# PickNikRobotics/pick_ik

Measured on AMD Instinct MI355X. Metric: converged IK solves/sec (7-DOF Panda, batched random targets), higher is better.
Workload: dtype f64; 1 GPU; panda 7-DOF memetic IK (BASELINE configs[1]): population 128, elites 4, batch 4096 random reachable targets per GPU per step, seed = ready pose, max_generations 100, gd_max_iters 25; robot=panda, dof=7, tip_frames=1, batch_per_gpu=4096, batches_per_call=64, calls=21, streams=4, problems_in_flight_per_gpu=1048576, parallelism=shard1, arithmetic=exact

## Files before the change

include/pick_ik_amd.h:

```cpp
#ifndef PICK_IK_AMD_H
#define PICK_IK_AMD_H

#include <stdint.h>

#ifdef __cplusplus
extern "C" {
#endif

#define PIKAMD_MAX_DOF 16

#define PIKAMD_SUCCESS 1
#define PIKAMD_APPROXIMATE 2
#define PIKAMD_NO_IK_SOLUTION (-31)

#define PIKAMD_EINVAL (-1)
#define PIKAMD_ENODEVICE (-2)
#define PIKAMD_EHIP (-3)
#define PIKAMD_EUNSUPPORTED (-4)

#define PIKAMD_JOINT_REVOLUTE 0
#define PIKAMD_JOINT_PRISMATIC 1
#define PIKAMD_JOINT_PLANAR_X 2
#define PIKAMD_JOINT_PLANAR_Y 3
#define PIKAMD_JOINT_PLANAR_THETA 4
#define PIKAMD_JOINT_FLOATING_TX 5
#define PIKAMD_JOINT_FLOATING_TY 6
#define PIKAMD_JOINT_FLOATING_TZ 7
#define PIKAMD_JOINT_FLOATING_RX 8
#define PIKAMD_JOINT_FLOATING_RY 9
#define PIKAMD_JOINT_FLOATING_RZ 10
#define PIKAMD_JOINT_FLOATING_RW 11

typedef struct pikamd_chain {
    int32_t dof;
    const double* origin_xyz_rpy;
    const double* axis;
    const int32_t* joint_type;
    const double* tip_xyz_rpy;
    const double* qmin;
    const double* qmax;
    const double* vmax;
    const uint8_t* bounded;
} pikamd_chain;

#define PIKAMD_MAX_TIPS 8
typedef struct pikamd_tip {
    int32_t n_joints;
    const int32_t* variable;
    const double* origin_xyz_rpy;
    const double* axis;
    const int32_t* joint_type;
    const double* tip_xyz_rpy;
} pikamd_tip;
typedef struct pikamd_multi_chain {
    int32_t dof;
    int32_t n_tips;
    const pikamd_tip* tips;
    const double* qmin;
    const double* qmax;
    const double* vmax;
    const uint8_t* bounded;
} pikamd_multi_chain;

typedef struct pikamd_params {
    int32_t mode;
    double gd_step_size;
    int32_t gd_max_iters;
    double gd_min_cost_delta;
    double position_threshold;
    double orientation_threshold;
    double cost_threshold;
    double position_scale;
    double rotation_scale;
    double center_joints_weight;
    double avoid_joint_limits_weight;
    double minimal_displacement_weight;
    int32_t stop_optimization_on_valid_solution;
    int32_t memetic_num_threads;
    int32_t memetic_stop_on_first_solution;
    int32_t memetic_population_size;
    int32_t memetic_elite_size;
    double memetic_wipeout_fitness_tol;
    int32_t memetic_max_generations;
    int32_t memetic_gd_max_iters;
    int32_t return_approximate_solution;
} pikamd_params;

typedef struct pikamd_stats {
    int64_t cost_evals;
    int32_t generations;
    int32_t wipeouts;
    int32_t pool_erasures;
    int32_t reserved;
} pikamd_stats;

typedef struct pikamd_solver pikamd_solver;

void pikamd_default_params(pikamd_params* p);

int32_t pikamd_create(const pikamd_chain* chain, int32_t device_ordinal, pikamd_solver** out);
int32_t pikamd_create_multi(const pikamd_multi_chain* chain, int32_t device_ordinal,
                            pikamd_solver** out);
int32_t pikamd_n_tips(const pikamd_solver* s);

#define PIKAMD_MAX_MIMIC 4
typedef struct pikamd_mimic_joint {
    int32_t tip;
    int32_t after_variable;
    int32_t master_variable;
    int32_t joint_type;
    double origin_xyz_rpy[6];
    double axis[3];
    double multiplier, offset;
} pikamd_mimic_joint;
int32_t pikamd_set_mimic_joints(pikamd_solver* s, int32_t n, const pikamd_mimic_joint* joints);
void pikamd_destroy(pikamd_solver* s);
int32_t pikamd_variables(const pikamd_solver* s, double* out);

int32_t pikamd_fk_batch(pikamd_solver* s, int64_t n, const double* q, double* pos_quat);

int32_t pikamd_cost_batch(pikamd_solver* s, const pikamd_params* p, int64_t n,
                          const double* goal_pos_quat, const double* seed, const double* q,
                          double* cost, int32_t* is_solution);

int32_t pikamd_gd_step_batch(pikamd_solver* s, const pikamd_params* p, int64_t n,
                             const double* goal_pos_quat, const double* seed, double* local,
                             double* best, double* local_cost, double* best_cost,
                             double* gradient, int32_t* improved);

int32_t pikamd_solve_batch(pikamd_solver* s, const pikamd_params* p, int64_t B,
                           const double* goal_pos_quat, const double* seed, uint64_t rng_seed,
                           int64_t problem_offset, double* solution, int32_t* status,
                           double* final_cost, pikamd_stats* stats);

#define PIKAMD_MAX_SLOTS 128
int32_t pikamd_solve_batch_device(pikamd_solver* s, const pikamd_params* p, int64_t B,
                                  const double* d_goal_pos_quat, const double* d_seed,
                                  uint64_t rng_seed, int64_t problem_offset, double* d_solution,
                                  int32_t* d_status, double* d_final_cost, pikamd_stats* d_stats,
                                  void* stream, int32_t slot);
int32_t pikamd_fk_batch_device(pikamd_solver* s, int64_t n, const double* d_q, double* d_pos_quat,
                               void* stream);
int32_t pikamd_reserve(pikamd_solver* s, const pikamd_params* p, int64_t B, int32_t slot,
                       void* stream);

#define PIKAMD_MAX_BATCHES 64
typedef struct pikamd_batch {
    int64_t B;
    const double* goal_pos_quat;
    const double* seed;
    const double* initial_guess;
    int64_t problem_offset;
    double* solution;
    int32_t* status;
    double* final_cost;
    pikamd_stats* stats;
    uint32_t* completed;
} pikamd_batch;

int32_t pikamd_solve_batches_device(pikamd_solver* s, const pikamd_params* p, int32_t n_batches,
                                    const pikamd_batch* batches, uint64_t rng_seed, void* stream,
                                    int32_t slot);

#define PIKAMD_MAX_HOST_JOBS 16
int32_t pikamd_solve_batches_async(pikamd_solver* s, const pikamd_params* p, int32_t n_batches,
                                   const pikamd_batch* batches, uint64_t rng_seed, int32_t job);
int32_t pikamd_wait(pikamd_solver* s, int32_t job);
int32_t pikamd_solve_batches(pikamd_solver* s, const pikamd_params* p, int32_t n_batches,
                             const pikamd_batch* batches, uint64_t rng_seed);

void pikamd_shard_bounds(int64_t total, int32_t rank, int32_t world, int64_t* lo, int64_t* hi);
int32_t pikamd_solve_batch_sharded(pikamd_solver* const* solvers, int32_t n_devices, const pikamd_params* p,
                                   int64_t B, const double* goal_pos_quat, const double* seed,
                                   const double* initial_guess , uint64_t rng_seed,
                                   int64_t problem_offset, double* solution, int32_t* status,
                                   double* final_cost , pikamd_stats* stats );

#define PIKAMD_MAX_NAME 64
typedef struct pikamd_urdf_model {
    int32_t dof, n_tips;
    char variable_names[PIKAMD_MAX_DOF][PIKAMD_MAX_NAME];
    double qmin[PIKAMD_MAX_DOF], qmax[PIKAMD_MAX_DOF], vmax[PIKAMD_MAX_DOF];
    uint8_t bounded[PIKAMD_MAX_DOF];
    struct {
        int32_t n_joints;
        int32_t variable[PIKAMD_MAX_DOF];
        double origin_xyz_rpy[PIKAMD_MAX_DOF][6];
        double axis[PIKAMD_MAX_DOF][3];
        int32_t joint_type[PIKAMD_MAX_DOF];
        double tip_xyz_rpy[6];
    } tips[PIKAMD_MAX_TIPS];
    int32_t n_mimic;
    pikamd_mimic_joint mimic[PIKAMD_MAX_TIPS * PIKAMD_MAX_MIMIC];
} pikamd_urdf_model;
int32_t pikamd_urdf_extract(const char* urdf_xml, const char* base_link, const char* const* tip_links,
                            int32_t n_tips, pikamd_urdf_model* out);
int32_t pikamd_create_from_urdf(const char* urdf_xml, const char* base_link, const char* const* tip_links,
                                int32_t n_tips, int32_t device_ordinal, pikamd_solver** out);

typedef double (*pikamd_cost_fn)(const double* q, int32_t dof, int32_t pose_index, void* user);
int32_t pikamd_solve_batch_host(pikamd_solver* s, const pikamd_params* p, int64_t B, const double* goal_pos_quat,
                                const double* seed, const double* initial_guess, uint64_t rng_seed,
                                int64_t problem_offset, pikamd_cost_fn cost_fn, void* user, double* solution,
                                int32_t* status, double* final_cost, pikamd_stats* stats);

int32_t pikamd_set_option(pikamd_solver* s, const char* name, const char* value);

int32_t pikamd_self_test(pikamd_solver* s, const pikamd_params* p, int32_t n, uint32_t* disabled_mask);
int32_t pikamd_self_test_cost(const pikamd_solver* s, int32_t* runs, double* total_ms);

const char* pikamd_last_error(void);
const char* pikamd_version(void);
const char* pikamd_kernel_name(const pikamd_solver* s, const pikamd_params* p);

#define PIKAMD_NOT_ATTEMPTED 0
#define PIKAMD_PATH_JUMP (-1001)
int32_t pikamd_solve_paths(pikamd_solver* s, const pikamd_params* p, int64_t P, int32_t W,
                           const double* goal_pos_quat, const double* start, const double* max_joint_step,
                           double* solution, int32_t* status, double* final_cost, pikamd_stats* stats,
                           int32_t* reached);
int32_t pikamd_solve_paths_device(pikamd_solver* s, const pikamd_params* p, int64_t P, int32_t W,
                                  const double* d_goal_pos_quat, const double* d_start,
                                  const double* d_max_joint_step, double* d_solution, int32_t* d_status,
                                  double* d_final_cost, pikamd_stats* d_stats, int32_t* d_reached,
                                  void* stream, int32_t slot);
const char* pikamd_path_kernel_name(const pikamd_solver* s, const pikamd_params* p, int64_t P);

#define PIKAMD_MAX_ATTEMPTS 64
int32_t pikamd_search_batch(pikamd_solver* s, const pikamd_params* p, int64_t B, const double* goal_pos_quat,
                            const double* seed, const double* initial_guess, uint64_t rng_seed,
                            int64_t problem_offset, int32_t max_attempts, double* solution, int32_t* status,
                            double* final_cost, pikamd_stats* stats, int32_t* attempts, double* all_solution,
                            int32_t* all_status);
int32_t pikamd_search_batch_device(pikamd_solver* s, const pikamd_params* p, int64_t B,
                                   const double* d_goal_pos_quat, const double* d_seed,
                                   const double* d_initial_guess, uint64_t rng_seed, int64_t problem_offset,
                                   int32_t max_attempts, double* d_solution, int32_t* d_status,
                                   double* d_final_cost, pikamd_stats* d_stats, int32_t* d_attempts,
                                   double* d_all_solution, int32_t* d_all_status, void* stream, int32_t slot);
const char* pikamd_search_kernel_name(const pikamd_solver* s, const pikamd_params* p, int64_t B,
                                      int32_t max_attempts, int32_t* attempts_in_flight);

#ifdef __cplusplus
}
#endif
#endif
```

pick_ik_amd/build.py:

```python
from __future__ import annotations

import concurrent.futures as cf
import hashlib
import os
import re
import shutil
import subprocess

_HERE = os.path.dirname(os.path.abspath(__file__))
CSRC = os.path.join(_HERE, "csrc")
LIB = os.path.join(_HERE, "libpick_ik_amd.so")
LIB_STRICT = os.path.join(_HERE, "libpick_ik_amd_strict.so")
HEADERS = ["pik_kernels.hpp", "pik_math.hpp", "pik_host.hpp", "pik_solver.hpp", "pik_launch.hpp", "pik_exact.hpp",
           "pik_host_solve.hpp", "pik_path.hpp", "pik_path_ops.hpp", "pik_search.hpp", "pik_search_ops.hpp"]
HEADER = os.path.join(os.path.dirname(_HERE), "include", "pick_ik_amd.h")
DOFS = tuple(range(1, 17))
BUILD_DIR = os.path.join(_HERE, "_build")


def hipcc() -> str:
    for cand in (shutil.which("hipcc"), "/opt/rocm/bin/hipcc"):
        if cand and os.path.exists(cand):
            return cand
    raise RuntimeError("hipcc not found")


COMMON_FLAGS = ["-DPIK_COMMON=1"]
COMMON_GOALS_FLAGS = ["-DPIK_COMMON=1", "-DPIK_NO_GOALS=0"]


def _flavor_flags(strict: bool):
    flags = ["-DPIK_STRICT=1", "-ffp-contract=off"] if strict else ["-ffp-contract=on"]
    return flags + os.environ.get("PIK_EXTRA_HIPCC_FLAGS", "").split()


def _objects(strict: bool):
    d = os.path.join(BUILD_DIR, "strict" if strict else "fast")
    only = os.environ.get("PIK_ONLY_D")
    keep = {int(x) for x in only.split(",")} if only else set(DOFS)
    objs = [(os.path.join(d, "pik_amd.o"), "pik_amd.hip", [])]
    objs.append((os.path.join(d, "pik_host_solve.o"), "pik_host_solve.hip",
                 ["--cuda-host-only"] + ([] if strict else EXACT_FLAGS)))
    for n in DOFS:
        extra = [f"-DPIK_INST_D={n}"] + ([] if n in keep else ["-DPIK_INST_STUB=1"])
        objs.append((os.path.join(d, f"pik_inst_d{n}.o"), "pik_inst.hip", extra))
    return objs


def _is_strict_obj(o) -> bool:
    return os.sep + "strict" + os.sep in o[0]


EXACT_FLAGS = ["-DPIK_STRICT=1", "-DPIK_EXACT_FMA=1", "-ffp-contract=off"]


def _exact_objects():
    d = os.path.join(BUILD_DIR, "exact")
    only = os.environ.get("PIK_ONLY_D")
    keep = {int(x) for x in only.split(",")} if only else set(DOFS)
    return [(os.path.join(d, f"pik_inst_d{n}.o"), "pik_inst.hip",
             [f"-DPIK_INST_D={n}"] + (EXACT_FLAGS if n in keep else ["-DPIK_INST_STUB=1"] + EXACT_FLAGS)) for n in DOFS]


def _is_exact_obj(o) -> bool:
    return os.sep + "exact" + os.sep in o[0]


def _path_objects(flavour: str):
    d = os.path.join(BUILD_DIR, flavour)
    fl = EXACT_FLAGS if flavour == "exact" else []
    only = os.environ.get("PIK_ONLY_D")
    keep = {int(x) for x in only.split(",")} if only else set(DOFS)
    return [(os.path.join(d, f"pik_path_inst_d{n}.o"), "pik_path_inst.hip",
             [f"-DPIK_INST_D={n}"] + (fl if n in keep else ["-DPIK_INST_STUB=1"] + fl)) for n in DOFS]


def _search_objects(flavour: str):
    d = os.path.join(BUILD_DIR, flavour)
    fl = EXACT_FLAGS if flavour == "exact" else []
    only = os.environ.get("PIK_ONLY_D")
    keep = {int(x) for x in only.split(",")} if only else set(DOFS)
    return [(os.path.join(d, f"pik_search_inst_d{n}.o"), "pik_search_inst.hip",
             [f"-DPIK_INST_D={n}"] + (fl if n in keep else ["-DPIK_INST_STUB=1"] + fl)) for n in DOFS]


def _common_objects(goals: bool = False):
    d = os.path.join(BUILD_DIR, "common_goals" if goals else "common")
    fl = COMMON_GOALS_FLAGS if goals else COMMON_FLAGS
    only = os.environ.get("PIK_ONLY_D")
    keep = {int(x) for x in only.split(",")} if only else set(DOFS)
    return [(os.path.join(d, f"pik_inst_d{n}.o"), "pik_inst.hip",
             [f"-DPIK_INST_D={n}"] + (fl if n in keep else ["-DPIK_INST_STUB=1"] + fl)) for n in DOFS]


def _cmd(obj, src, extra, strict):
    bare = "-DPIK_EXACT_FMA=1" in extra
    flavour = os.environ.get("PIK_EXTRA_HIPCC_FLAGS", "").split() if bare else _flavor_flags(strict)
    return [hipcc(), "--offload-arch=gfx950", "--offload-compress", "-O2", "-std=c++17", "-fPIC", "-c", *flavour,
            "-Rpass-analysis=kernel-resource-usage", *extra, "-o", obj, os.path.join(CSRC, src)]


def _stamp(cmd):
    return hashlib.sha1(" ".join(cmd).encode()).hexdigest()


def _obj_stale(obj, src, extra, strict) -> bool:
    if not os.path.exists(obj) or not os.path.exists(obj + ".cmd"):
        return True
    if open(obj + ".cmd").read() != _stamp(_cmd(obj, src, extra, strict)):
        return True
    deps = _deps(src, "-DPIK_STRICT=1" in _cmd(obj, src, extra, strict))
    if os.path.exists(obj + ".deps"):
        return open(obj + ".deps").read() != _code_hash(deps)
    t = os.path.getmtime(obj)
    if any(os.path.getmtime(d) > t for d in deps):
        return True
    with open(obj + ".deps", "w") as f:
        f.write(_code_hash(deps))
    return False


def _strip_comments(text: str) -> str:
    out, i, n = [], 0, len(text)
    while i < n:
        c = text[i]
        if c == '"' or c == "'":
            j = i + 1
            while j < n and text[j] != c:
                j += 2 if text[j] == "\\" else 1
            out.append(text[i:j + 1])
            i = j + 1
        elif text.startswith("//", i):
            j = text.find("\n", i)
            i = n if j < 0 else j
        elif text.startswith("/*", i):
            j = text.find("*/", i + 2)
            i = n if j < 0 else j + 2
            out.append(" ")
        else:
            out.append(c)
            i += 1
    return " ".join("".join(out).split())


_code_hash_cache = {}


def _code_hash(files) -> str:
    h = hashlib.sha1()
    for f in files:
        key = (f, os.path.getmtime(f))
        if key not in _code_hash_cache:
            _code_hash_cache[key] = hashlib.sha1(_strip_comments(open(f).read()).encode()).hexdigest()
        h.update(_code_hash_cache[key].encode())
    return h.hexdigest()


_INCLUDE = re.compile(r'^\s*#\s*include\s+"([^"]+)"', re.M)


def _deps(src, strict_flags: bool):
    seen, todo = [], [os.path.join(CSRC, src)]
    while todo:
        f = os.path.realpath(todo.pop())
        if f in seen or not os.path.exists(f):
            continue
        seen.append(f)
        for inc in _INCLUDE.findall(open(f).read()):
            if os.path.basename(inc) == "pik_exact.hpp" and not strict_flags:
                continue
            todo.append(os.path.join(os.path.dirname(f), inc))
    return seen


def _sources():
    return ([os.path.join(CSRC, f) for f in ("pik_amd.hip", "pik_inst.hip", "pik_path_inst.hip", "pik_search_inst.hip", "pik_urdf.hpp",
                                             *HEADERS)] +
            [HEADER, os.path.abspath(__file__)])


def _lib_stamp(strict: bool) -> str:
    flags = _flavor_flags(strict) + ([] if strict else ["+exact:"] + EXACT_FLAGS + ["+common:"] + COMMON_FLAGS + ["+common_goals:"] + COMMON_GOALS_FLAGS)
    return _stamp(flags + ["+paths", "+search", "only=" + os.environ.get("PIK_ONLY_D", "all")])


def is_stale(lib: str = LIB) -> bool:
    if not os.path.exists(lib) or not os.path.exists(lib + ".stamp"):
        return True
    if open(lib + ".stamp").read() != _lib_stamp(lib == LIB_STRICT):
        return True
    t = os.path.getmtime(lib)
    return any(os.path.getmtime(d) > t for d in _sources())


def _compile(obj, src, extra, strict, verbose):
    os.makedirs(os.path.dirname(obj), exist_ok=True)
    cmd = _cmd(obj, src, extra, strict)
    if verbose:
        print(" ".join(cmd), flush=True)
    r = subprocess.run(cmd, cwd=CSRC, stderr=subprocess.PIPE, text=True)
    if r.returncode != 0:
        raise RuntimeError(f"{' '.join(cmd)}\n{r.stderr[-4000:]}")
    with open(obj + ".res", "w") as f:
        f.write(r.stderr)
    with open(obj + ".cmd", "w") as f:
        f.write(_stamp(cmd))
    with open(obj + ".deps", "w") as f:
        f.write(_code_hash(_deps(src, "-DPIK_STRICT=1" in cmd)))


def _link(lib, objs, verbose):
    cmd = [hipcc(), "--offload-arch=gfx950", "-shared", "-fPIC", "-o", lib + ".tmp", *objs]
    if verbose:
        print(" ".join(cmd), flush=True)
    subprocess.run(cmd, check=True)
    os.replace(lib + ".tmp", lib)


FLAVOUR_FLAGS = {
    "pik": ["-ffp-contract=on"],
    "pik_common": ["-ffp-contract=on"] + COMMON_FLAGS,
    "pik_common_goals": ["-ffp-contract=on"] + COMMON_GOALS_FLAGS,
    "pik_exact": EXACT_FLAGS,
    "pik_strict": ["-DPIK_STRICT=1", "-ffp-contract=off"],
}
_flavour_sha_cache = {}


def _host_api_lines():
    out, inside = set(), False
    for n, line in enumerate(open(HEADER).read().splitlines(), 1):
        if "[host-api-begin]" in line:
            inside = True
        if inside:
            out.add(n)
        if "[host-api-end]" in line:
            inside = False
    return out


def flavour_sha(namespace: str, dof: int = 7) -> str:
    key = (namespace, dof)
    if key in _flavour_sha_cache:
        return _flavour_sha_cache[key]
    flags = FLAVOUR_FLAGS[namespace]
    cmd = [hipcc(), "--offload-arch=gfx950", "-std=c++17", "--cuda-device-only", "-E", *flags, f"-DPIK_INST_D={dof}",
           os.path.join(CSRC, "pik_inst.hip"), "-o", "-"]
    r = subprocess.run(cmd, cwd=CSRC, stdout=subprocess.PIPE, stderr=subprocess.PIPE, text=True)
    if r.returncode != 0:
        raise RuntimeError(f"{' '.join(cmd)}\n{r.stderr[-2000:]}")
    own = (os.path.realpath(CSRC) + os.sep, os.path.realpath(HEADER))
    host_api = _host_api_lines()
    h = hashlib.sha256(" ".join(flags).encode())
    keep, in_header, lineno = False, False, 0
    for line in r.stdout.splitlines():
        if line.startswith("# ") and '"' in line:
            f = line.split('"')[1]
            rp = os.path.realpath(f if os.path.isabs(f) else os.path.join(CSRC, f))
            keep = rp.startswith(own[0]) or rp == own[1]
            in_header = rp == own[1]
            lineno = int(line.split()[1])
            continue
        if keep and line.strip() and not (in_header and lineno in host_api):
            h.update(line.strip().encode())
            h.update(b"\n")
        lineno += 1
    _flavour_sha_cache[key] = h.hexdigest()[:16]
    return _flavour_sha_cache[key]


LEDGER = os.path.join(BUILD_DIR, "kernel_resources.csv")


def ledger_rows():
    from . import kernel_resources as KR
    rows = []
    for o in (_objects(False) + _exact_objects() + _common_objects() + _common_objects(True) + _objects(True) +
              _path_objects("fast") + _path_objects("exact") + _path_objects("strict") +
              _search_objects("fast") + _search_objects("exact") + _search_objects("strict")):
        res = o[0] + ".res"
        if o[1] not in ("pik_inst.hip", "pik_path_inst.hip", "pik_search_inst.hip"):
            continue
        if not os.path.exists(res):
            return None
        flavour = os.path.basename(os.path.dirname(o[0]))
        rows += KR.rows_of(open(res).read(), flavour)
    return rows


def write_ledger(path: str = LEDGER):
    from . import kernel_resources as KR
    rows = ledger_rows()
    if rows is None:
        return None
    os.makedirs(os.path.dirname(path), exist_ok=True)
    with open(path, "w") as f:
        f.write("flavour,kernel," + ",".join(KR.FIELDS) + "\n")
        for fl, name, v in sorted(rows, key=lambda r: (r[0], r[1])):
            f.write(f'{fl},"{name}",' + ",".join(str(v[k]) for k in KR.FIELDS) + "\n")
    return path


def build_jobs() -> int:
    if os.environ.get("MAX_JOBS", "").isdigit() and int(os.environ["MAX_JOBS"]) > 0:
        return int(os.environ["MAX_JOBS"])
    try:
        return max(1, len(os.sched_getaffinity(0)))
    except AttributeError:
        return max(1, os.cpu_count() or 1)


def build_library(force: bool = False, verbose: bool = False, strict_too: bool = True) -> str:
    flavors = [(LIB, False)] + ([(LIB_STRICT, True)] if strict_too else [])
    jobs, relink = [], []
    for lib, strict in flavors:
        if not (force or is_stale(lib) or os.environ.get("PIK_ONLY_D") or os.environ.get("PIK_EXTRA_HIPCC_FLAGS")):
            continue
        objs = _objects(strict)
        if not strict:
            objs = objs + _exact_objects() + _common_objects() + _common_objects(True)
        objs = objs + (_path_objects("strict") if strict else _path_objects("fast") + _path_objects("exact"))
        objs = objs + (_search_objects("strict") if strict else _search_objects("fast") + _search_objects("exact"))
        stale = [o for o in objs if force or _obj_stale(*o, _is_strict_obj(o))]
        jobs += [(o, _is_strict_obj(o)) for o in stale if (o, _is_strict_obj(o)) not in jobs]
        relink.append((lib, [o[0] for o in objs]))
    if jobs:
        def length_of(job):
            for fl in job[0][2]:
                if fl.startswith("-DPIK_INST_D="):
                    return -int(fl.split("=")[1])
            return -100
        jobs.sort(key=length_of)
        with cf.ThreadPoolExecutor(max_workers=build_jobs()) as ex:
            for f in [ex.submit(_compile, *o, strict, verbose) for o, strict in jobs]:
                f.result()
    for lib, objs in relink:
        _link(lib, objs, verbose)
        with open(lib + ".stamp", "w") as f:
            f.write(_lib_stamp(lib == LIB_STRICT))
    if relink and not os.environ.get("PIK_ONLY_D"):
        write_ledger()
    return LIB


if __name__ == "__main__":
    import sys
    if "--ledger" in sys.argv:
        build_library()
        print(write_ledger(sys.argv[sys.argv.index("--ledger") + 1]))
    else:
        print(build_library(force="--force" in sys.argv, verbose=True, strict_too="--fast-only" not in sys.argv))
```

pick_ik_amd/csrc/pik_amd.hip:

```cpp
#include <hip/hip_runtime.h>

#include <chrono>
#include <cmath>
#include <cstdlib>
#include <memory>
#include <new>
#include <string>
#include <thread>
#include <vector>

#include "pik_path_ops.hpp"
#include "pik_search_ops.hpp"
#include "pik_solver.hpp"
#include "pik_urdf.hpp"

namespace pik {
char* error_buffer() {
    static thread_local char buf[ERROR_BUFFER_SIZE] = "";
    return buf;
}
}

using pik::fail;

#if !defined(PIK_STRICT)
namespace pik_exact {
char* error_buffer() { return ::pik::error_buffer(); }
#define PIK_LITERAL_OPS(N) const void* launch_ops_d##N();
PIK_LITERAL_OPS(1) PIK_LITERAL_OPS(2) PIK_LITERAL_OPS(3) PIK_LITERAL_OPS(4) PIK_LITERAL_OPS(5) PIK_LITERAL_OPS(6)
PIK_LITERAL_OPS(7) PIK_LITERAL_OPS(8) PIK_LITERAL_OPS(9) PIK_LITERAL_OPS(10) PIK_LITERAL_OPS(11) PIK_LITERAL_OPS(12)
PIK_LITERAL_OPS(13) PIK_LITERAL_OPS(14) PIK_LITERAL_OPS(15) PIK_LITERAL_OPS(16)
#undef PIK_LITERAL_OPS
#define PIK_LITERAL_PATH_OPS(N) const void* path_ops_d##N();
PIK_LITERAL_PATH_OPS(1) PIK_LITERAL_PATH_OPS(2) PIK_LITERAL_PATH_OPS(3) PIK_LITERAL_PATH_OPS(4)
PIK_LITERAL_PATH_OPS(5) PIK_LITERAL_PATH_OPS(6) PIK_LITERAL_PATH_OPS(7) PIK_LITERAL_PATH_OPS(8)
PIK_LITERAL_PATH_OPS(9) PIK_LITERAL_PATH_OPS(10) PIK_LITERAL_PATH_OPS(11) PIK_LITERAL_PATH_OPS(12)
PIK_LITERAL_PATH_OPS(13) PIK_LITERAL_PATH_OPS(14) PIK_LITERAL_PATH_OPS(15) PIK_LITERAL_PATH_OPS(16)
#undef PIK_LITERAL_PATH_OPS
#define PIK_LITERAL_SEARCH_OPS(N) const void* search_ops_d##N();
PIK_LITERAL_SEARCH_OPS(1) PIK_LITERAL_SEARCH_OPS(2) PIK_LITERAL_SEARCH_OPS(3) PIK_LITERAL_SEARCH_OPS(4)
PIK_LITERAL_SEARCH_OPS(5) PIK_LITERAL_SEARCH_OPS(6) PIK_LITERAL_SEARCH_OPS(7) PIK_LITERAL_SEARCH_OPS(8)
PIK_LITERAL_SEARCH_OPS(9) PIK_LITERAL_SEARCH_OPS(10) PIK_LITERAL_SEARCH_OPS(11) PIK_LITERAL_SEARCH_OPS(12)
PIK_LITERAL_SEARCH_OPS(13) PIK_LITERAL_SEARCH_OPS(14) PIK_LITERAL_SEARCH_OPS(15) PIK_LITERAL_SEARCH_OPS(16)
#undef PIK_LITERAL_SEARCH_OPS
}
namespace pik_common {
char* error_buffer() { return ::pik::error_buffer(); }
#define PIK_COMMON_OPS(N) const void* launch_ops_d##N();
PIK_COMMON_OPS(1) PIK_COMMON_OPS(2) PIK_COMMON_OPS(3) PIK_COMMON_OPS(4) PIK_COMMON_OPS(5) PIK_COMMON_OPS(6)
PIK_COMMON_OPS(7) PIK_COMMON_OPS(8) PIK_COMMON_OPS(9) PIK_COMMON_OPS(10) PIK_COMMON_OPS(11) PIK_COMMON_OPS(12)
PIK_COMMON_OPS(13) PIK_COMMON_OPS(14) PIK_COMMON_OPS(15) PIK_COMMON_OPS(16)
#undef PIK_COMMON_OPS
}
namespace pik_common_goals {
char* error_buffer() { return ::pik::error_buffer(); }
#define PIK_COMMON_OPS(N) const void* launch_ops_d##N();
PIK_COMMON_OPS(1) PIK_COMMON_OPS(2) PIK_COMMON_OPS(3) PIK_COMMON_OPS(4) PIK_COMMON_OPS(5) PIK_COMMON_OPS(6)
PIK_COMMON_OPS(7) PIK_COMMON_OPS(8) PIK_COMMON_OPS(9) PIK_COMMON_OPS(10) PIK_COMMON_OPS(11) PIK_COMMON_OPS(12)
PIK_COMMON_OPS(13) PIK_COMMON_OPS(14) PIK_COMMON_OPS(15) PIK_COMMON_OPS(16)
#undef PIK_COMMON_OPS
}
#endif

namespace {

struct SolverExt : pikamd_solver {
    int search_schedule = pik::SEARCH_ADAPTIVE;
    pik::DevBuf search_rows[pik::N_SLOTS];
};
SolverExt* ext_of(pikamd_solver* s) { return static_cast<SolverExt*>(s); }
const SolverExt* ext_of(const pikamd_solver* s) { return static_cast<const SolverExt*>(s); }

#if !defined(PIK_STRICT)
const pik::LaunchOps* literal_ops(int dof) {
    const void* p = nullptr;
    switch (dof) {
#define PIK_LITERAL_CASE(N) case N: p = pik_exact::launch_ops_d##N(); break;
        PIK_LITERAL_CASE(1) PIK_LITERAL_CASE(2) PIK_LITERAL_CASE(3) PIK_LITERAL_CASE(4) PIK_LITERAL_CASE(5)
        PIK_LITERAL_CASE(6) PIK_LITERAL_CASE(7) PIK_LITERAL_CASE(8) PIK_LITERAL_CASE(9) PIK_LITERAL_CASE(10)
        PIK_LITERAL_CASE(11) PIK_LITERAL_CASE(12) PIK_LITERAL_CASE(13) PIK_LITERAL_CASE(14) PIK_LITERAL_CASE(15)
        PIK_LITERAL_CASE(16)
#undef PIK_LITERAL_CASE
        default: break;
    }
    return static_cast<const pik::LaunchOps*>(p);
}
#endif

#if !defined(PIK_STRICT)
const pik::LaunchOps* common_ops(int dof, bool goals = false) {
    const void* p = nullptr;
    switch (dof) {
#define PIK_COMMON_CASE(N) case N: p = goals ? pik_common_goals::launch_ops_d##N() : pik_common::launch_ops_d##N(); break;
        PIK_COMMON_CASE(1) PIK_COMMON_CASE(2) PIK_COMMON_CASE(3) PIK_COMMON_CASE(4) PIK_COMMON_CASE(5)
        PIK_COMMON_CASE(6) PIK_COMMON_CASE(7) PIK_COMMON_CASE(8) PIK_COMMON_CASE(9) PIK_COMMON_CASE(10)
        PIK_COMMON_CASE(11) PIK_COMMON_CASE(12) PIK_COMMON_CASE(13) PIK_COMMON_CASE(14) PIK_COMMON_CASE(15)
        PIK_COMMON_CASE(16)
#undef PIK_COMMON_CASE
        default: break;
    }
    return static_cast<const pik::LaunchOps*>(p);
}
#endif

int check_solver(const pikamd_solver* s) {
    if (!s) return fail(PIKAMD_EINVAL, "solver handle is NULL");
    return 0;
}

[[maybe_unused]] bool needs_literal(const pikamd_solver* s) {
    bool f = s->opt.exact || s->chain.float_mask != 0u || s->chain.n_mimic != 0;
    for (int k = 1; k < s->n_tips; ++k) f = f || s->more[k - 1].float_mask != 0u || s->more[k - 1].n_mimic != 0;
    return f;
}
[[maybe_unused]] bool needs_literal(const pikamd_solver* s, const pikamd_params* p) {
    return needs_literal(s) || (p && p->gd_step_size > 1.0e-2);
}
const pik::LaunchOps* ops_of(const pikamd_solver* s, const pikamd_params* p = nullptr) {
#if !defined(PIK_STRICT)
    if (needs_literal(s, p)) return literal_ops(s->chain.dof);
#else
    (void)p;
#endif
    return pik::launch_ops(s->chain.dof);
}

[[maybe_unused]] bool common_eligible(const pikamd_solver* s, const pikamd_params* p, const pik::ParamsK& pk) {
    if (!s->opt.specialised || needs_literal(s)) return false;
    const uint32_t all = (s->chain.dof >= 32) ? ~0u : ((1u << s->chain.dof) - 1u);
    auto chain_ok = [&](const pik::ChainHost& c) {
        return c.prismatic_mask == 0u && c.dh_general_mask == 0u && c.bounded_mask == all;
    };
    if (!chain_ok(s->chain)) return false;
    for (int k = 1; k < s->n_tips; ++k)
        if (!chain_ok(s->more[k - 1])) return false;
    if (pk.line_delta == 0 || !(pk.pos_scale > 0.0) || !(pk.rot_scale > 0.0)) return false;
    if (p->mode == 0 && (pk.elites != 4 || p->memetic_num_threads > 1)) return false;
    return true;
}
const pik::LaunchOps* solve_ops_of(const pikamd_solver* s, const pikamd_params* p, const pik::ParamsK& pk) {
#if !defined(PIK_STRICT)
    if (common_eligible(s, p, pk))
        if (const pik::LaunchOps* o = common_ops(s->chain.dof, pk.goal_mask != 0)) return o;
#else
    (void)pk;
#endif
    return ops_of(s, p);
}

int no_kernels(int dof) {
    return fail(PIKAMD_EUNSUPPORTED, "dof %d: kernels are instantiated for 1..16", dof);
}

const pik::PathOps* path_ops_of(const pikamd_solver* s, const pikamd_params* p) {
#if !defined(PIK_STRICT)
    if (needs_literal(s, p)) {
        const void* o = nullptr;
        switch (s->chain.dof) {
#define PIK_LITERAL_PATH_CASE(N) case N: o = pik_exact::path_ops_d##N(); break;
            PIK_LITERAL_PATH_CASE(1) PIK_LITERAL_PATH_CASE(2) PIK_LITERAL_PATH_CASE(3) PIK_LITERAL_PATH_CASE(4)
            PIK_LITERAL_PATH_CASE(5) PIK_LITERAL_PATH_CASE(6) PIK_LITERAL_PATH_CASE(7) PIK_LITERAL_PATH_CASE(8)
            PIK_LITERAL_PATH_CASE(9) PIK_LITERAL_PATH_CASE(10) PIK_LITERAL_PATH_CASE(11) PIK_LITERAL_PATH_CASE(12)
            PIK_LITERAL_PATH_CASE(13) PIK_LITERAL_PATH_CASE(14) PIK_LITERAL_PATH_CASE(15) PIK_LITERAL_PATH_CASE(16)
#undef PIK_LITERAL_PATH_CASE
            default: break;
        }
        return static_cast<const pik::PathOps*>(o);
    }
#else
    (void)p;
#endif
    return pik::path_ops(s->chain.dof);
}

const pik::SearchOps* search_ops_of(const pikamd_solver* s, const pikamd_params* p) {
#if !defined(PIK_STRICT)
    if (needs_literal(s, p)) {
        const void* o = nullptr;
        switch (s->chain.dof) {
#define PIK_LITERAL_SEARCH_CASE(N) case N: o = pik_exact::search_ops_d##N(); break;
            PIK_LITERAL_SEARCH_CASE(1) PIK_LITERAL_SEARCH_CASE(2) PIK_LITERAL_SEARCH_CASE(3) PIK_LITERAL_SEARCH_CASE(4)
            PIK_LITERAL_SEARCH_CASE(5) PIK_LITERAL_SEARCH_CASE(6) PIK_LITERAL_SEARCH_CASE(7) PIK_LITERAL_SEARCH_CASE(8)
            PIK_LITERAL_SEARCH_CASE(9) PIK_LITERAL_SEARCH_CASE(10) PIK_LITERAL_SEARCH_CASE(11) PIK_LITERAL_SEARCH_CASE(12)
            PIK_LITERAL_SEARCH_CASE(13) PIK_LITERAL_SEARCH_CASE(14) PIK_LITERAL_SEARCH_CASE(15) PIK_LITERAL_SEARCH_CASE(16)
#undef PIK_LITERAL_SEARCH_CASE
            default: break;
        }
        return static_cast<const pik::SearchOps*>(o);
    }
#else
    (void)p;
#endif
    return pik::search_ops(s->chain.dof);
}

size_t align8(size_t v) { return (v + 7) & ~(size_t)7; }

}

extern "C" {

void pikamd_default_params(pikamd_params* p) {
    if (!p) return;
    p->mode = 0;
    p->gd_step_size = 0.0001;
    p->gd_max_iters = 100;
    p->gd_min_cost_delta = 1.0e-12;
    p->position_threshold = 0.001;
    p->orientation_threshold = 0.001;
    p->cost_threshold = 0.001;
    p->position_scale = 1.0;
    p->rotation_scale = 0.5;
    p->center_joints_weight = 0.0;
    p->avoid_joint_limits_weight = 0.0;
    p->minimal_displacement_weight = 0.0;
    p->stop_optimization_on_valid_solution = 1;
    p->memetic_num_threads = 1;
    p->memetic_stop_on_first_solution = 1;
    p->memetic_population_size = 16;
    p->memetic_elite_size = 4;
    p->memetic_wipeout_fitness_tol = 0.00001;
    p->memetic_max_generations = 100;
    p->memetic_gd_max_iters = 25;
    p->return_approximate_solution = 0;
}

const char* pikamd_last_error(void) { return pik::error_buffer(); }

const char* pikamd_version(void) { return "pick_ik_amd 0.3.0 (gfx950)"; }

static int32_t create_solver(const pik::ChainHost* chains, int n_tips, int32_t device_ordinal,
                             pikamd_solver** out) {
    int count = 0;
    if (hipGetDeviceCount(&count) != hipSuccess || count < 1)
        return fail(PIKAMD_ENODEVICE, "no HIP device available (this library has no CPU path)");
    if (device_ordinal < 0 || device_ordinal >= count)
        return fail(PIKAMD_EINVAL, "device_ordinal %d out of range [0, %d)", device_ordinal, count);
    if (!pik::launch_ops(chains[0].dof)) return no_kernels(chains[0].dof);
    HIP_TRY(hipSetDevice(device_ordinal));
    hipDeviceProp_t prop;
    HIP_TRY(hipGetDeviceProperties(&prop, device_ordinal));
    pikamd_solver* s = new (std::nothrow) SolverExt();
    if (!s) return fail(PIKAMD_EHIP, "out of host memory");
    s->device = device_ordinal;
    s->num_cu = prop.multiProcessorCount;
    s->chain = chains[0];
    s->n_tips = n_tips;
    for (int k = 1; k < n_tips; ++k) s->more[k - 1] = chains[k];
    const size_t table_bytes = sizeof(pik::BatchRecord) * PIKAMD_MAX_BATCHES * pik::TABLE_RING;
    hipError_t e = hipMalloc(reinterpret_cast<void**>(&s->counters), pik::COUNTER_BLOCK * pik::N_SLOTS);
    if (e == hipSuccess) e = hipMemset(s->counters, 0, pik::COUNTER_BLOCK * pik::N_SLOTS);
    if (e == hipSuccess) e = hipMalloc(reinterpret_cast<void**>(&s->consts_dev), pik::CONSTS_STRIDE * pik::N_SLOTS);
    if (e == hipSuccess)
        e = hipHostMalloc(reinterpret_cast<void**>(&s->consts_host), pik::CONSTS_STRIDE * pik::N_SLOTS, hipHostMallocDefault);
    if (e == hipSuccess) e = hipMalloc(reinterpret_cast<void**>(&s->tables_dev), table_bytes);
    if (e == hipSuccess) e = hipHostMalloc(reinterpret_cast<void**>(&s->tables_host), table_bytes, hipHostMallocDefault);
    for (int i = 0; i < pik::TABLE_RING && e == hipSuccess; ++i)
        e = hipEventCreateWithFlags(&s->table_event[i], hipEventDisableTiming);
    if (e != hipSuccess) {
        pikamd_destroy(s);
        return fail(PIKAMD_EHIP, "device allocation failed: %s", hipGetErrorString(e));
    }
    for (auto& j : s->jobs) j.host.pinned_host = true;
    *out = s;
    return 0;
}

int32_t pikamd_create(const pikamd_chain* chain, int32_t device_ordinal, pikamd_solver** out) {
    if (!out) return fail(PIKAMD_EINVAL, "out is NULL");
    *out = nullptr;
    pik::ChainHost ch;
    if (const char* msg = pik::build_chain(chain, ch)) return fail(PIKAMD_EINVAL, "%s", msg);
    return create_solver(&ch, 1, device_ordinal, out);
}

int32_t pikamd_create_multi(const pikamd_multi_chain* chain, int32_t device_ordinal,
                            pikamd_solver** out) {
    if (!out) return fail(PIKAMD_EINVAL, "out is NULL");
    *out = nullptr;
    if (!chain || !chain->tips) return fail(PIKAMD_EINVAL, "multi-tip chain is NULL");
    if (chain->n_tips < 1 || chain->n_tips > PIKAMD_MAX_TIPS)
        return fail(PIKAMD_EINVAL, "n_tips %d out of range [1, %d]", chain->n_tips, PIKAMD_MAX_TIPS);
    if (!chain->qmin || !chain->qmax) return fail(PIKAMD_EINVAL, "chain has NULL arrays");
    std::vector<pik::ChainHost> ch((size_t)chain->n_tips);
    uint32_t used = 0;
    for (int k = 0; k < chain->n_tips; ++k) {
        if (const char* msg = pik::build_tip_chain(chain, k, ch[k])) return fail(PIKAMD_EINVAL, "tip %d: %s", k, msg);
        used |= ch[k].active_mask;
    }
    if (used != ((chain->dof >= 32) ? ~0u : ((1u << chain->dof) - 1u)))
        return fail(PIKAMD_EINVAL, "a variable is on no tip's path");
    return create_solver(ch.data(), chain->n_tips, device_ordinal, out);
}

int32_t pikamd_urdf_extract(const char* urdf_xml, const char* base_link, const char* const* tip_links,
                            int32_t n_tips, pikamd_urdf_model* out) {
    if (!out) return fail(PIKAMD_EINVAL, "out is NULL");
    const std::string err = pik::urdf::extract(urdf_xml, base_link, tip_links, n_tips, *out);
    if (!err.empty()) return fail(PIKAMD_EINVAL, "%s", err.c_str());
    return 0;
}

int32_t pikamd_create_from_urdf(const char* urdf_xml, const char* base_link, const char* const* tip_links,
                                int32_t n_tips, int32_t device_ordinal, pikamd_solver** out) {
    if (!out) return fail(PIKAMD_EINVAL, "out is NULL");
    *out = nullptr;
    auto m = std::make_unique<pikamd_urdf_model>();
    if (int rc = pikamd_urdf_extract(urdf_xml, base_link, tip_links, n_tips, m.get())) return rc;
    if (m->n_tips == 1) {
        const auto& t = m->tips[0];
        pikamd_chain c{m->dof, &t.origin_xyz_rpy[0][0], &t.axis[0][0], t.joint_type, t.tip_xyz_rpy,
                       m->qmin,  m->qmax,               m->vmax,       m->bounded};
        if (int rc = pikamd_create(&c, device_ordinal, out)) return rc;
        if (m->n_mimic)
            if (int rc = pikamd_set_mimic_joints(*out, m->n_mimic, m->mimic)) {
                pikamd_destroy(*out);
                *out = nullptr;
                return rc;
            }
        return 0;
    }
    pikamd_tip tips[PIKAMD_MAX_TIPS];
    for (int k = 0; k < m->n_tips; ++k) {
        const auto& t = m->tips[k];
        tips[k] = pikamd_tip{t.n_joints, t.variable, &t.origin_xyz_rpy[0][0], &t.axis[0][0], t.joint_type, t.tip_xyz_rpy};
    }
    pikamd_multi_chain c{m->dof, m->n_tips, tips, m->qmin, m->qmax, m->vmax, m->bounded};
    if (int rc = pikamd_create_multi(&c, device_ordinal, out)) return rc;
    if (m->n_mimic)
        if (int rc = pikamd_set_mimic_joints(*out, m->n_mimic, m->mimic)) {
            pikamd_destroy(*out);
            *out = nullptr;
            return rc;
        }
    return 0;
}

int32_t pikamd_n_tips(const pikamd_solver* s) { return s ? s->n_tips : 0; }

int32_t pikamd_set_mimic_joints(pikamd_solver* s, int32_t n, const pikamd_mimic_joint* joints) {
    if (int rc = check_solver(s)) return rc;
    if (n < 0 || (n > 0 && !joints)) return fail(PIKAMD_EINVAL, "bad arguments");
    pik::ChainHost saved[PIKAMD_MAX_TIPS];
    for (int k = 0; k < s->n_tips; ++k) saved[k] = k == 0 ? s->chain : s->more[k - 1];
    auto path = [&](int k) -> pik::ChainHost& { return k == 0 ? s->chain : s->more[k - 1]; };
    for (int k = 0; k < s->n_tips; ++k) pik::clear_mimic_joints(path(k));
    for (int i = 0; i < n; ++i) {
        const pikamd_mimic_joint& m = joints[i];
        const char* msg = (m.tip < 0 || m.tip >= s->n_tips) ? "mimic joint: tip out of range" : pik::add_mimic_joint(path(m.tip), m);
        if (!msg && s->n_tips > 1) {
            const uint32_t act = path(m.tip).active_mask;
            if (!((act >> m.master_variable) & 1u) || (m.after_variable >= 0 && !((act >> m.after_variable) & 1u)))
                msg = "mimic joint: master_variable / after_variable is not on that tip's path";
        }
        if (msg) {
            for (int k = 0; k < s->n_tips; ++k) path(k) = saved[k];
            return fail(PIKAMD_EINVAL, "%s", msg);
        }
    }
    s->self_tested.clear();
    s->opt.disabled_lanes = 0;
    s->opt.disabled_lanes_exact = 0;
    return 0;
}

void pikamd_destroy(pikamd_solver* s) {
    if (!s) return;
    (void)hipSetDevice(s->device);
    (void)hipDeviceSynchronize();
    if (s->counters) (void)hipFree(s->counters);
    if (s->consts_dev) (void)hipFree(s->consts_dev);
    if (s->consts_host) (void)hipHostFree(s->consts_host);
    if (s->tables_dev) (void)hipFree(s->tables_dev);
    if (s->tables_host) (void)hipHostFree(s->tables_host);
    for (auto& ev : s->table_event)
        if (ev) (void)hipEventDestroy(ev);
    for (auto& ev : s->slot_event)
        if (ev) (void)hipEventDestroy(ev);
    for (auto& b : s->stage) b.release();
    for (auto& b : s->slot_state) b.release();
    for (auto& b : s->slot_soa) b.release();
    for (auto& b : ext_of(s)->search_rows) b.release();
    for (auto& j : s->jobs) {
        j.dev.release();
        j.host.release();
        if (j.stream) (void)hipStreamDestroy(j.stream);
    }
    delete ext_of(s);
}

int32_t pikamd_variables(const pikamd_solver* s, double* out) {
    if (int rc = check_solver(s)) return rc;
    if (!out) return fail(PIKAMD_EINVAL, "out is NULL");
    for (int j = 0; j < s->chain.dof; ++j) {
        out[7 * j + 0] = s->chain.qmin[j];
        out[7 * j + 1] = s->chain.qmax[j];
        out[7 * j + 2] = s->chain.mid[j];
        out[7 * j + 3] = s->chain.hspan[j];
        out[7 * j + 4] = s->chain.vrcp[j];
        out[7 * j + 5] = s->chain.mdf[j];
        out[7 * j + 6] = ((s->chain.bounded_mask >> j) & 1u) ? 1.0 : 0.0;
    }
    return 0;
}

int32_t pikamd_fk_batch_device(pikamd_solver* s, int64_t n, const double* d_q, double* d_pos_quat,
                               void* stream) {
    if (int rc = check_solver(s)) return rc;
    if (n < 0 || (n > 0 && (!d_q || !d_pos_quat))) return fail(PIKAMD_EINVAL, "bad arguments");
    HIP_TRY(hipSetDevice(s->device));
    return ops_of(s)->fk(s, n, d_q, d_pos_quat, (hipStream_t)stream);
}

int32_t pikamd_fk_batch(pikamd_solver* s, int64_t n, const double* q, double* pos_quat) {
    if (int rc = check_solver(s)) return rc;
    if (n < 0 || (n > 0 && (!q || !pos_quat))) return fail(PIKAMD_EINVAL, "bad arguments");
    if (n == 0) return 0;
    HIP_TRY(hipSetDevice(s->device));
    const size_t d = (size_t)s->chain.dof;
    if (int rc = s->stage[0].ensure(sizeof(double) * d * (size_t)n)) return rc;
    if (int rc = s->stage[1].ensure(sizeof(double) * 7 * (size_t)s->n_tips * (size_t)n)) return rc;
    HIP_TRY(hipMemcpy(s->stage[0].p, q, sizeof(double) * d * (size_t)n, hipMemcpyHostToDevice));
    if (int rc = pikamd_fk_batch_device(s, n, (const double*)s->stage[0].p, (double*)s->stage[1].p, nullptr))
        return rc;
    HIP_TRY(hipMemcpy(pos_quat, s->stage[1].p, sizeof(double) * 7 * (size_t)s->n_tips * (size_t)n, hipMemcpyDeviceToHost));
    return 0;
}

int32_t pikamd_cost_batch(pikamd_solver* s, const pikamd_params* p, int64_t n,
                          const double* goal_pos_quat, const double* seed, const double* q,
                          double* cost, int32_t* is_solution) {
    if (int rc = check_solver(s)) return rc;
    pik::ParamsK pk;
    if (!p) return fail(PIKAMD_EINVAL, "params is NULL");
    if (const char* msg = pik::make_params_k(p, pk)) {
        pikamd_params q2 = *p;
        q2.mode = 1;
        if (const char* m2 = pik::make_params_k(&q2, pk)) return fail(PIKAMD_EINVAL, "%s", m2);
        (void)msg;
    }
    if (n < 0 || (n > 0 && (!goal_pos_quat || !seed || !q))) return fail(PIKAMD_EINVAL, "bad arguments");
    if (n == 0) return 0;
    HIP_TRY(hipSetDevice(s->device));
    const size_t d = (size_t)s->chain.dof, N = (size_t)n;
    if (int rc = s->stage[0].ensure(sizeof(double) * 7 * (size_t)s->n_tips * N)) return rc;
    if (int rc = s->stage[1].ensure(sizeof(double) * d * N)) return rc;
    if (int rc = s->stage[2].ensure(sizeof(double) * d * N)) return rc;
    if (int rc = s->stage[3].ensure(sizeof(double) * N)) return rc;
    if (int rc = s->stage[4].ensure(sizeof(int) * N)) return rc;
    HIP_TRY(hipMemcpy(s->stage[0].p, goal_pos_quat, sizeof(double) * 7 * (size_t)s->n_tips * N, hipMemcpyHostToDevice));
    HIP_TRY(hipMemcpy(s->stage[1].p, seed, sizeof(double) * d * N, hipMemcpyHostToDevice));
    HIP_TRY(hipMemcpy(s->stage[2].p, q, sizeof(double) * d * N, hipMemcpyHostToDevice));
    if (int rc = ops_of(s)->cost(s, pk, n, (const double*)s->stage[0].p, (const double*)s->stage[1].p,
                                 (const double*)s->stage[2].p, cost ? (double*)s->stage[3].p : nullptr,
                                 is_solution ? (int*)s->stage[4].p : nullptr, nullptr))
        return rc;
    if (cost) HIP_TRY(hipMemcpy(cost, s->stage[3].p, sizeof(double) * N, hipMemcpyDeviceToHost));
    if (is_solution) HIP_TRY(hipMemcpy(is_solution, s->stage[4].p, sizeof(int) * N, hipMemcpyDeviceToHost));
    HIP_TRY(hipDeviceSynchronize());
    return 0;
}

int32_t pikamd_gd_step_batch(pikamd_solver* s, const pikamd_params* p, int64_t n,
                             const double* goal_pos_quat, const double* seed, double* local,
                             double* best, double* local_cost, double* best_cost,
                             double* gradient, int32_t* improved) {
    if (int rc = check_solver(s)) return rc;
    pik::ParamsK pk;
    pikamd_params q2;
    if (!p) return fail(PIKAMD_EINVAL, "params is NULL");
    q2 = *p;
    q2.mode = 1;
    if (const char* msg = pik::make_params_k(&q2, pk)) return fail(PIKAMD_EINVAL, "%s", msg);
    if (n < 0 || (n > 0 && (!goal_pos_quat || !seed || !local || !best || !local_cost || !best_cost || !gradient)))
        return fail(PIKAMD_EINVAL, "bad arguments");
    if (n == 0) return 0;
    HIP_TRY(hipSetDevice(s->device));
    const size_t d = (size_t)s->chain.dof, N = (size_t)n;
    const size_t sz[8] = {sizeof(double) * 7 * (size_t)s->n_tips * N, sizeof(double) * d * N, sizeof(double) * d * N,
                          sizeof(double) * d * N, sizeof(double) * N,     sizeof(double) * N,
                          sizeof(double) * d * N, sizeof(int) * N};
    for (int i = 0; i < 8; ++i)
        if (int rc = s->stage[i].ensure(sz[i])) return rc;
    HIP_TRY(hipMemcpy(s->stage[0].p, goal_pos_quat, sz[0], hipMemcpyHostToDevice));
    HIP_TRY(hipMemcpy(s->stage[1].p, seed, sz[1], hipMemcpyHostToDevice));
    HIP_TRY(hipMemcpy(s->stage[2].p, local, sz[2], hipMemcpyHostToDevice));
    HIP_TRY(hipMemcpy(s->stage[3].p, best, sz[3], hipMemcpyHostToDevice));
    HIP_TRY(hipMemcpy(s->stage[4].p, local_cost, sz[4], hipMemcpyHostToDevice));
    HIP_TRY(hipMemcpy(s->stage[5].p, best_cost, sz[5], hipMemcpyHostToDevice));
    if (int rc = ops_of(s, p)->step(s, pk, n, (const double*)s->stage[0].p, (const double*)s->stage[1].p,
                                 (double*)s->stage[2].p, (double*)s->stage[3].p, (double*)s->stage[4].p,
                                 (double*)s->stage[5].p, (double*)s->stage[6].p, (int*)s->stage[7].p, nullptr))
        return rc;
    HIP_TRY(hipMemcpy(local, s->stage[2].p, sz[2], hipMemcpyDeviceToHost));
    HIP_TRY(hipMemcpy(best, s->stage[3].p, sz[3], hipMemcpyDeviceToHost));
    HIP_TRY(hipMemcpy(local_cost, s->stage[4].p, sz[4], hipMemcpyDeviceToHost));
    HIP_TRY(hipMemcpy(best_cost, s->stage[5].p, sz[5], hipMemcpyDeviceToHost));
    HIP_TRY(hipMemcpy(gradient, s->stage[6].p, sz[6], hipMemcpyDeviceToHost));
    if (improved) HIP_TRY(hipMemcpy(improved, s->stage[7].p, sz[7], hipMemcpyDeviceToHost));
    HIP_TRY(hipDeviceSynchronize());
    return 0;
}



static int make_records(const pikamd_solver* s, int32_t n_batches, const pikamd_batch* batches,
                        pik::BatchRecord* rec, long long* total) {
    if (n_batches < 0 || n_batches > PIKAMD_MAX_BATCHES)
        return fail(PIKAMD_EINVAL, "n_batches %d out of range [0, %d]", n_batches, PIKAMD_MAX_BATCHES);
    if (n_batches > 0 && !batches) return fail(PIKAMD_EINVAL, "batches is NULL");
    long long sum = 0;
    int n = 0;
    for (int k = 0; k < n_batches; ++k) {
        const pikamd_batch& b = batches[k];
        if (b.B < 0 || (b.B > 0 && (!b.goal_pos_quat || !b.seed || !b.solution || !b.status)))
            return fail(PIKAMD_EINVAL, "batch %d: bad arguments", k);
        if (b.B == 0) continue;
        pik::BatchRecord& r = rec[n++];
        r.start = 0;
        r.B = b.B;
        r.goal = b.goal_pos_quat;
        r.seed = b.seed;
        r.guess = b.initial_guess ? b.initial_guess : b.seed;
        r.problem_offset = b.problem_offset;
        r.solution = b.solution;
        r.status = b.status;
        r.cost = b.final_cost;
        r.stats = b.stats;
        r.completed = b.completed;
        sum += b.B;
    }
    (void)s;
    *total = sum;
    return n;
}

__global__ void pik_joint_layout_kernel(const double* __restrict__ in, double* __restrict__ out, long long B, int D,
                                        int to_aos) {
    const long long i = (long long)blockIdx.x * blockDim.x + threadIdx.x;
    if (i >= B * D) return;
    if (to_aos) {
        const long long b = i / D;
        const int j = (int)(i - b * D);
        out[i] = in[(long long)j * B + b];
    } else {
        const long long j = i / B, b = i - j * B;
        out[i] = in[b * D + j];
    }
}

static int maybe_self_test(pikamd_solver* s, const pikamd_params* p);

static int32_t solve_records(pikamd_solver* s, const pikamd_params* p, pik::BatchRecord* rec, int n,
                             uint64_t rng_seed, hipStream_t stream, int slot) {
    pik::ParamsK pk;
    if (const char* msg = pik::make_params_k(p, pk)) return fail(PIKAMD_EINVAL, "%s", msg);
    if (n == 0) return 0;
    HIP_TRY(hipSetDevice(s->device));
    if (!s->opt.soa) return solve_ops_of(s, p, pk)->solve(s, p, pk, rec, n, rng_seed, stream, slot, false);
    const int D = s->chain.dof;
    size_t doubles = 0;
    for (int k = 0; k < n; ++k) {
        if (rec[k].completed)
            return fail(PIKAMD_EINVAL, "joint_layout soa: completion counters are not available (the solutions of a "
                                       "batch are in place when the stream has passed the call)");
        doubles += (size_t)rec[k].B * (size_t)D * (rec[k].guess != rec[k].seed ? 3u : 2u);
    }
    if (int rc = s->slot_soa[slot].ensure(sizeof(double) * doubles)) return rc;
    double* w = (double*)s->slot_soa[slot].p;
    double* user_solution[PIKAMD_MAX_BATCHES];
    auto move = [&](const double* in, double* out, long long B, int to_aos) -> int {
        const long long items = B * D;
        hipLaunchKernelGGL(pik_joint_layout_kernel, dim3((unsigned)((items + 255) / 256)), dim3(256), 0, stream, in, out, B,
                           D, to_aos);
        HIP_TRY(hipGetLastError());
        return 0;
    };
    for (int k = 0; k < n; ++k) {
        const long long B = rec[k].B;
        const bool own_guess = rec[k].guess != rec[k].seed;
        double* sd = w;
        w += (size_t)B * D;
        if (int rc = move(rec[k].seed, sd, B, 1)) return rc;
        double* gs = sd;
        if (own_guess) {
            gs = w;
            w += (size_t)B * D;
            if (int rc = move(rec[k].guess, gs, B, 1)) return rc;
        }
        user_solution[k] = rec[k].solution;
        rec[k].seed = sd;
        rec[k].guess = gs;
        rec[k].solution = w;
        w += (size_t)B * D;
    }
    if (int rc = solve_ops_of(s, p, pk)->solve(s, p, pk, rec, n, rng_seed, stream, slot, false)) return rc;
    for (int k = 0; k < n; ++k)
        if (int rc = move(rec[k].solution, user_solution[k], rec[k].B, 0)) return rc;
    return 0;
}

int32_t pikamd_solve_batches_device(pikamd_solver* s, const pikamd_params* p, int32_t n_batches,
                                    const pikamd_batch* batches, uint64_t rng_seed, void* stream,
                                    int32_t slot) {
    if (int rc = check_solver(s)) return rc;
    if (slot < 0 || slot >= PIKAMD_MAX_SLOTS) return fail(PIKAMD_EINVAL, "slot out of range");
    pik::BatchRecord rec[PIKAMD_MAX_BATCHES];
    long long total = 0;
    const int n = make_records(s, n_batches, batches, rec, &total);
    if (n < 0) return n;
    return solve_records(s, p, rec, n, rng_seed, (hipStream_t)stream, slot);
}

int32_t pikamd_solve_batch_device(pikamd_solver* s, const pikamd_params* p, int64_t B,
                                  const double* d_goal_pos_quat, const double* d_seed,
                                  uint64_t rng_seed, int64_t problem_offset, double* d_solution,
                                  int32_t* d_status, double* d_final_cost, pikamd_stats* d_stats,
                                  void* stream, int32_t slot) {
    const pikamd_batch b = {B,          d_goal_pos_quat, d_seed,       nullptr, problem_offset,
                            d_solution, d_status,        d_final_cost, d_stats, nullptr};
    return pikamd_solve_batches_device(s, p, 1, &b, rng_seed, stream, slot);
}

int32_t pikamd_reserve(pikamd_solver* s, const pikamd_params* p, int64_t B, int32_t slot, void* stream) {
    if (int rc = check_solver(s)) return rc;
    pik::ParamsK pk;
    if (const char* msg = pik::make_params_k(p, pk)) return fail(PIKAMD_EINVAL, "%s", msg);
    if (B < 0) return fail(PIKAMD_EINVAL, "bad arguments");
    if (slot < 0 || slot >= PIKAMD_MAX_SLOTS) return fail(PIKAMD_EINVAL, "slot out of range");
    if (B == 0) return 0;
    if (int rc = maybe_self_test(s, p)) return rc;
    HIP_TRY(hipSetDevice(s->device));
    if (s->opt.soa)
        if (int rc = s->slot_soa[slot].ensure(sizeof(double) * (size_t)B * (size_t)s->chain.dof * 3u)) return rc;
    pik::BatchRecord rec;
    std::memset(&rec, 0, sizeof rec);
    rec.B = B;
    return solve_ops_of(s, p, pk)->solve(s, p, pk, &rec, 1, 0, (hipStream_t)stream, slot, true);
}

static int32_t start_job(pikamd_solver* s, const pikamd_params* p, int32_t n_batches,
                         const pikamd_batch* batches, uint64_t rng_seed, int job) {
    if (int rc = check_solver(s)) return rc;
    if (job < 0 || job > pik::JOB_SELF_TEST) return fail(PIKAMD_EINVAL, "job out of range");
    if (job != pik::JOB_SELF_TEST)
        if (int rc = maybe_self_test(s, p)) return rc;
    pik::HostJob& J = s->jobs[job];
    if (J.pending) return fail(PIKAMD_EINVAL, "job %d is still in flight: call pikamd_wait first", job);
    pik::BatchRecord rec[PIKAMD_MAX_BATCHES];
    long long total = 0;
    const int n = make_records(s, n_batches, batches, rec, &total);
    if (n < 0) return n;
    {
        pik::ParamsK pk;
        if (const char* msg = pik::make_params_k(p, pk)) return fail(PIKAMD_EINVAL, "%s", msg);
    }
    J.n_batches = 0;
    if (n == 0) return 0;
    HIP_TRY(hipSetDevice(s->device));
    if (!J.stream) HIP_TRY(hipStreamCreateWithFlags(&J.stream, hipStreamNonBlocking));
    const size_t d = (size_t)s->chain.dof, g7 = 7 * (size_t)s->n_tips;
    size_t off = 0;
    size_t in_goal[PIKAMD_MAX_BATCHES], in_seed[PIKAMD_MAX_BATCHES], in_guess[PIKAMD_MAX_BATCHES];
    for (int k = 0; k < n; ++k) {
        const size_t N = (size_t)rec[k].B;
        in_goal[k] = off;
        off += sizeof(double) * g7 * N;
        in_seed[k] = off;
        off += sizeof(double) * d * N;
        in_guess[k] = (rec[k].guess != rec[k].seed) ? off : in_seed[k];
        if (rec[k].guess != rec[k].seed) off += sizeof(double) * d * N;
    }
    J.in_bytes = off;
    for (int k = 0; k < n; ++k) {
        const size_t N = (size_t)rec[k].B;
        pik::HostJob::Out& o = J.outs[k];
        o.B = rec[k].B;
        o.solution = rec[k].solution;
        o.status = rec[k].status;
        o.final_cost = rec[k].cost;
        o.stats = (pikamd_stats*)rec[k].stats;
        o.off_solution = off;
        off += sizeof(double) * d * N;
        o.off_cost = off;
        off += sizeof(double) * N;
        o.off_stats = off;
        off += sizeof(pikamd_stats) * N;
        o.off_status = off;
        off += align8(sizeof(int32_t) * N);
    }
    J.out_bytes = off - J.in_bytes;
    if (int rc = J.dev.ensure(off)) return rc;
    if (int rc = J.host.ensure(off)) return rc;
    char* hb = (char*)J.host.p;
    char* db = (char*)J.dev.p;
    for (int k = 0; k < n; ++k) {
        const size_t N = (size_t)rec[k].B;
        std::memcpy(hb + in_goal[k], rec[k].goal, sizeof(double) * g7 * N);
        std::memcpy(hb + in_seed[k], rec[k].seed, sizeof(double) * d * N);
        if (in_guess[k] != in_seed[k]) std::memcpy(hb + in_guess[k], rec[k].guess, sizeof(double) * d * N);
        rec[k].goal = (const double*)(db + in_goal[k]);
        rec[k].seed = (const double*)(db + in_seed[k]);
        rec[k].guess = (const double*)(db + in_guess[k]);
        rec[k].solution = (double*)(db + J.outs[k].off_solution);
        rec[k].status = (int*)(db + J.outs[k].off_status);
        rec[k].cost = (double*)(db + J.outs[k].off_cost);
        rec[k].stats = (void*)(db + J.outs[k].off_stats);
        rec[k].completed = nullptr;
    }
    HIP_TRY(hipMemcpyAsync(db, hb, J.in_bytes, hipMemcpyHostToDevice, J.stream));
    if (int rc = solve_records(s, p, rec, n, rng_seed, J.stream, pik::N_DEVICE_SLOTS + job)) {
        (void)hipStreamSynchronize(J.stream);
        return rc;
    }
    {
        const hipError_t e = hipMemcpyAsync(hb + J.in_bytes, db + J.in_bytes, J.out_bytes, hipMemcpyDeviceToHost, J.stream);
        if (e != hipSuccess) {
            (void)hipStreamSynchronize(J.stream);
            return fail(PIKAMD_EHIP, "result copy could not be enqueued: %s", hipGetErrorString(e));
        }
    }
    J.n_batches = n;
    J.dof = (int)d;
    J.pending = true;
    return 0;
}

int32_t pikamd_solve_batches_async(pikamd_solver* s, const pikamd_params* p, int32_t n_batches,
                                   const pikamd_batch* batches, uint64_t rng_seed, int32_t job) {
    if (job < 0 || job >= PIKAMD_MAX_HOST_JOBS - 1)
        return fail(PIKAMD_EINVAL, "job out of range [0, %d)", PIKAMD_MAX_HOST_JOBS - 1);
    return start_job(s, p, n_batches, batches, rng_seed, job);
}

static int32_t wait_job(pikamd_solver* s, int job) {
    pik::HostJob& J = s->jobs[job];
    if (!J.pending) return 0;
    HIP_TRY(hipSetDevice(s->device));
    {
        const hipError_t e = hipStreamSynchronize(J.stream);
        J.pending = false;
        if (e != hipSuccess) return fail(PIKAMD_EHIP, "job %d: %s (its results are lost)", job, hipGetErrorString(e));
    }
    const char* hb = (const char*)J.host.p;
    const size_t d = (size_t)J.dof;
    for (int k = 0; k < J.n_batches; ++k) {
        const pik::HostJob::Out& o = J.outs[k];
        const size_t N = (size_t)o.B;
        std::memcpy(o.solution, hb + o.off_solution, sizeof(double) * d * N);
        std::memcpy(o.status, hb + o.off_status, sizeof(int32_t) * N);
        if (o.final_cost) std::memcpy(o.final_cost, hb + o.off_cost, sizeof(double) * N);
        if (o.stats) std::memcpy(o.stats, hb + o.off_stats, sizeof(pikamd_stats) * N);
    }
    return 0;
}

int32_t pikamd_wait(pikamd_solver* s, int32_t job) {
    if (int rc = check_solver(s)) return rc;
    if (job < 0 || job >= pik::N_HOST_JOBS) return fail(PIKAMD_EINVAL, "job out of range");
    return wait_job(s, job);
}

int32_t pikamd_solve_batches(pikamd_solver* s, const pikamd_params* p, int32_t n_batches,
                             const pikamd_batch* batches, uint64_t rng_seed) {
    const int job = PIKAMD_MAX_HOST_JOBS - 1;
    if (int rc = start_job(s, p, n_batches, batches, rng_seed, job)) return rc;
    return pikamd_wait(s, job);
}

int32_t pikamd_solve_batch(pikamd_solver* s, const pikamd_params* p, int64_t B,
                           const double* goal_pos_quat, const double* seed, uint64_t rng_seed,
                           int64_t problem_offset, double* solution, int32_t* status,
                           double* final_cost, pikamd_stats* stats) {
    const pikamd_batch b = {B,        goal_pos_quat, seed,       nullptr, problem_offset,
                            solution, status,        final_cost, stats,   nullptr};
    const int job = PIKAMD_MAX_HOST_JOBS - 1;
    if (int rc = start_job(s, p, 1, &b, rng_seed, job)) return rc;
    return pikamd_wait(s, job);
}

int32_t pikamd_set_option(pikamd_solver* s, const char* name, const char* value) {
    if (int rc = check_solver(s)) return rc;
    if (!name) return fail(PIKAMD_EINVAL, "option name is NULL");
    const std::string n = name, v = value ? value : "";
    pik::SolverOptions& o = s->opt;
    auto ints = [](const std::string& text, char sep, std::vector<int>& out) {
        size_t i = 0;
        while (i < text.size()) {
            char* end = nullptr;
            const long x = std::strtol(text.c_str() + i, &end, 10);
            if (end == text.c_str() + i) return false;
            out.push_back((int)x);
            i = (size_t)(end - text.c_str());
            if (i < text.size()) {
                if (text[i] != sep) return false;
                ++i;
            }
        }
        return true;
    };
    if (n == "lanes_per_elite") {
        if (v.empty()) { o.lpe = 0; return 0; }
        std::vector<int> x;
        if (!ints(v, ',', x) || x.size() != 1 || !(x[0] == 0 || x[0] == 1 || x[0] == 2 || x[0] == 4 || x[0] == 8 || x[0] == 16))
            return fail(PIKAMD_EINVAL, "lanes_per_elite: expected 0 (adaptive), 1, 2, 4, 8 or 16, got '%s'", v.c_str());
        o.lpe = x[0];
        return 0;
    }
    if (n == "lanes_per_elite_schedule") {
        if (v.empty()) { o.n_sched = 0; return 0; }
        int cnt = 0, from[4], of[4];
        size_t i = 0;
        while (i < v.size()) {
            const size_t comma = v.find(',', i), colon = v.find(':', i);
            const size_t end = comma == std::string::npos ? v.size() : comma;
            std::vector<int> a, b;
            if (cnt >= 4 || colon == std::string::npos || colon > end || !ints(v.substr(i, colon - i), ',', a) ||
                !ints(v.substr(colon + 1, end - colon - 1), ',', b) || a.size() != 1 || b.size() != 1 ||
                !(b[0] == 1 || b[0] == 2 || b[0] == 4 || b[0] == 8 || b[0] == 16) ||
                (cnt == 0 ? a[0] != 0 : a[0] <= from[cnt - 1]))
                return fail(PIKAMD_EINVAL, "lanes_per_elite_schedule: expected 'g0:l0,g1:l1,...' with g0 = 0, ascending "
                                           "generations and lanes in {1,2,4,8,16} (at most 4 entries), got '%s'", v.c_str());
            from[cnt] = a[0];
            of[cnt] = b[0];
            ++cnt;
            i = end + (end < v.size() ? 1 : 0);
        }
        o.n_sched = cnt;
        for (int k = 0; k < cnt; ++k) o.sched_from[k] = from[k], o.sched_of[k] = of[k];
        return 0;
    }
    if (n == "passes") {
        if (v.empty()) { o.passes_set = false; return 0; }
        std::vector<int> x;
        if (v != "none" && (!ints(v, ',', x) || x.size() > 15))
            return fail(PIKAMD_EINVAL, "passes: expected 'none' or up to 15 ascending generation marks, got '%s'", v.c_str());
        for (size_t k = 0; k < x.size(); ++k)
            if (x[k] <= 0 || (k > 0 && x[k] <= x[k - 1]))
                return fail(PIKAMD_EINVAL, "passes: marks must be positive and ascending, got '%s'", v.c_str());
        o.passes_set = true;
        o.n_marks = (int)x.size();
        for (size_t k = 0; k < x.size(); ++k) o.marks[k] = x[k];
        return 0;
    }
    if (n == "two_per_simd") {
        if (v.empty()) { o.two_per_simd = -1; return 0; }
        std::vector<int> x;
        if (!ints(v, ',', x) || x.size() != 1 || x[0] < 0)
            return fail(PIKAMD_EINVAL, "two_per_simd: expected 0, 1 or a wavefront threshold, got '%s'", v.c_str());
        o.two_per_simd = x[0];
        return 0;
    }
    if (n == "arithmetic") {
#if defined(PIK_STRICT)
        if (v.empty() || v == "exact") return 0;
        return fail(PIKAMD_EINVAL, "arithmetic: the verification library only has 'exact', got '%s'", v.c_str());
#else
        if (v.empty() || v == "exact") { o.exact = true; return 0; }
        if (v == "fast") { o.exact = false; return 0; }
        return fail(PIKAMD_EINVAL, "arithmetic: expected 'fast' or 'exact', got '%s'", v.c_str());
#endif
    }
    if (n == "self_test") {
        if (v.empty() || v == "auto") { o.auto_self_test = true; return 0; }
        if (v == "off") { o.auto_self_test = false; return 0; }
        return fail(PIKAMD_EINVAL, "self_test: expected 'auto' or 'off', got '%s'", v.c_str());
    }
    if (n == "specialised") {
        if (v.empty() || v == "1") { o.specialised = true; return 0; }
        if (v == "0") { o.specialised = false; return 0; }
        return fail(PIKAMD_EINVAL, "specialised: expected '0' or '1', got '%s'", v.c_str());
    }
    if (n == "shard_chunks") {
        if (v.empty()) { o.shard_chunks = 0; return 0; }
        std::vector<int> x;
        if (!ints(v, ',', x) || x.size() != 1 || x[0] < 1 || x[0] > 8)
            return fail(PIKAMD_EINVAL, "shard_chunks: expected 1..8, got '%s'", v.c_str());
        o.shard_chunks = x[0];
        return 0;
    }
    if (n == "joint_layout") {
        if (v.empty() || v == "aos") { o.soa = false; return 0; }
        if (v == "soa") { o.soa = true; return 0; }
        return fail(PIKAMD_EINVAL, "joint_layout: expected 'aos' or 'soa', got '%s'", v.c_str());
    }
    if (n == "host_max_time" || n == "host_gd_max_time") {
        double x = 0.0;
        if (!v.empty()) {
            char* end = nullptr;
            x = std::strtod(v.c_str(), &end);
            if (end == v.c_str() || *end != 0 || !(x >= 0.0) || !std::isfinite(x))
                return fail(PIKAMD_EINVAL, "%s: expected a time in seconds >= 0, got '%s'", n.c_str(), v.c_str());
        }
        (n == "host_max_time" ? o.host_max_time : o.host_gd_max_time) = x;
        return 0;
    }
    if (n == "search_schedule") {
        int& sched = ext_of(s)->search_schedule;
        if (v.empty() || v == "adaptive") { sched = pik::SEARCH_ADAPTIVE; return 0; }
        if (v == "sequential") { sched = pik::SEARCH_SEQUENTIAL; return 0; }
        if (v == "parallel") { sched = pik::SEARCH_PARALLEL; return 0; }
        return fail(PIKAMD_EINVAL, "search_schedule: expected 'adaptive', 'sequential' or 'parallel', got '%s'", v.c_str());
    }
    if (n == "regime") {
        if (v.empty() || v == "adaptive") { o.regime = 0; return 0; }
        if (v == "latency") { o.regime = 1; return 0; }
        if (v == "throughput") { o.regime = 2; return 0; }
        return fail(PIKAMD_EINVAL, "regime: expected 'adaptive', 'latency' or 'throughput', got '%s'", v.c_str());
    }
    return fail(PIKAMD_EINVAL, "unknown option '%s'", n.c_str());
}


void pikamd_shard_bounds(int64_t total, int32_t rank, int32_t world, int64_t* lo, int64_t* hi) {
    if (world < 1) world = 1;
    if (total < 0) total = 0;
    const int64_t base = total / world, rem = total % world;
    const int64_t l = (int64_t)rank * base + (rank < rem ? rank : rem);
    if (lo) *lo = l;
    if (hi) *hi = l + base + (rank < rem ? 1 : 0);
}

int32_t pikamd_solve_batch_sharded(pikamd_solver* const* solvers, int32_t n_devices, const pikamd_params* p,
                                   int64_t B, const double* goal_pos_quat, const double* seed,
                                   const double* initial_guess, uint64_t rng_seed, int64_t problem_offset,
                                   double* solution, int32_t* status, double* final_cost, pikamd_stats* stats) {
    if (!solvers || n_devices < 1) return fail(PIKAMD_EINVAL, "no solver handles");
    if (B < 0 || (B > 0 && (!goal_pos_quat || !seed || !solution || !status))) return fail(PIKAMD_EINVAL, "bad arguments");
    for (int r = 0; r < n_devices; ++r) {
        if (!solvers[r]) return fail(PIKAMD_EINVAL, "solver handle %d is NULL", r);
        if (solvers[r]->chain.dof != solvers[0]->chain.dof || solvers[r]->n_tips != solvers[0]->n_tips)
            return fail(PIKAMD_EINVAL, "solver handle %d describes a different chain", r);
        for (int q = 0; q < r; ++q)
            if (solvers[q] == solvers[r]) return fail(PIKAMD_EINVAL, "solver handle %d is given twice", r);
    }
    if (B == 0) return 0;
    for (int r = 0; r < n_devices; ++r)
        if (solvers[r]->opt.soa)
            return fail(PIKAMD_EINVAL, "joint_layout soa: not with pikamd_solve_batch_sharded (a shard of a [dof][B] "
                                       "array is not contiguous)");
    const size_t d = (size_t)solvers[0]->chain.dof, g7 = 7 * (size_t)solvers[0]->n_tips;
    constexpr int MAX_CHUNKS = 2;
    constexpr int64_t CHUNK_MIN = 32768;
    std::vector<int> rc((size_t)n_devices, 0);
    std::vector<std::string> msg((size_t)n_devices);
    auto work = [&](int r) {
        int64_t lo = 0, hi = 0;
        pikamd_shard_bounds(B, r, n_devices, &lo, &hi);
        const int64_t n = hi - lo;
        if (n == 0) return;
        int chunks = (int)((n + CHUNK_MIN - 1) / CHUNK_MIN);
        const int max_chunks = solvers[r]->opt.shard_chunks > 0 ? solvers[r]->opt.shard_chunks : MAX_CHUNKS;
        chunks = chunks < 1 ? 1 : chunks > max_chunks ? max_chunks : chunks;
        int started = 0;
        for (int c = 0; c < chunks && rc[r] == 0; ++c) {
            int64_t clo = 0, chi = 0;
            pikamd_shard_bounds(n, c, chunks, &clo, &chi);
            const int64_t a = lo + clo;
            const pikamd_batch b = {chi - clo,
                                    goal_pos_quat + (size_t)a * g7,
                                    seed + (size_t)a * d,
                                    initial_guess ? initial_guess + (size_t)a * d : nullptr,
                                    problem_offset + a,
                                    solution + (size_t)a * d,
                                    status + a,
                                    final_cost ? final_cost + a : nullptr,
                                    stats ? stats + a : nullptr,
                                    nullptr};
            rc[r] = pikamd_solve_batches_async(solvers[r], p, 1, &b, rng_seed, c);
            if (rc[r] == 0) ++started;
        }
        for (int c = 0; c < started; ++c) {
            const int w = pikamd_wait(solvers[r], c);
            if (rc[r] == 0) rc[r] = w;
        }
        if (rc[r] != 0) msg[r] = pik::error_buffer();
    };
    if (n_devices == 1) {
        work(0);
    } else {
        std::vector<std::thread> th;
        th.reserve((size_t)n_devices);
        for (int r = 0; r < n_devices; ++r) th.emplace_back(work, r);
        for (auto& t : th) t.join();
    }
    for (int r = 0; r < n_devices; ++r)
        if (rc[r] != 0) return fail(rc[r], "device shard %d: %s", r, msg[r].c_str());
    return 0;
}

#if defined(PIK_STRICT)
#define PIK_HOST_SOLVE pik_strict_host_solve
#else
#define PIK_HOST_SOLVE pik_exact_host_solve
#endif
}
extern "C" int PIK_HOST_SOLVE(const pikamd_solver* s, const pikamd_params* p, long long B, const double* goal,
                              const double* seed, const double* guess, unsigned long long rng_seed,
                              long long problem_offset, pikamd_cost_fn cb, void* user, double* solution, int32_t* status,
                              double* final_cost, pikamd_stats* stats);
extern "C" {

int32_t pikamd_solve_batch_host(pikamd_solver* s, const pikamd_params* p, int64_t B, const double* goal_pos_quat,
                                const double* seed, const double* initial_guess, uint64_t rng_seed,
                                int64_t problem_offset, pikamd_cost_fn cost_fn, void* user, double* solution,
                                int32_t* status, double* final_cost, pikamd_stats* stats) {
    if (int rc = check_solver(s)) return rc;
    if (!p) return fail(PIKAMD_EINVAL, "params is NULL");
    if (!cost_fn)
        return fail(PIKAMD_EINVAL, "pikamd_solve_batch_host is for queries with a host cost function; without one "
                                   "use pikamd_solve_batch (the GPU)");
    if (B < 0 || (B > 0 && (!goal_pos_quat || !seed || !solution || !status))) return fail(PIKAMD_EINVAL, "bad arguments");
    if (p->mode == 0 && (p->memetic_elite_size < 1 || p->memetic_population_size <= p->memetic_elite_size))
        return fail(PIKAMD_EINVAL, "memetic_population_size must exceed memetic_elite_size >= 1");
    if (s->opt.soa)
        return fail(PIKAMD_EINVAL, "joint_layout soa: not with pikamd_solve_batch_host (its arrays are [B][dof])");
    return PIK_HOST_SOLVE(s, p, B, goal_pos_quat, seed, initial_guess, rng_seed, problem_offset, cost_fn, user, solution,
                          status, final_cost, stats);
}

int32_t pikamd_self_test(pikamd_solver* s, const pikamd_params* p, int32_t n, uint32_t* disabled_out) {
    if (int rc = check_solver(s)) return rc;
    if (!p) return fail(PIKAMD_EINVAL, "params is NULL");
    if (n < 1 || n > 4096) return fail(PIKAMD_EINVAL, "n out of range [1, 4096]");
    const bool exact_now = pik::EXACT_FLAVOUR || s->opt.exact || needs_literal(s, p);
    auto mask_of = [exact_now](pik::SolverOptions& o) -> unsigned& { return exact_now ? o.disabled_lanes_exact : o.disabled_lanes; };
    if (disabled_out) *disabled_out = mask_of(s->opt);
    const int d = s->chain.dof, tips = s->n_tips;
    std::vector<double> q((size_t)n * d), goal((size_t)n * 7 * tips), seed((size_t)n * d);
    unsigned long long x = 0x9E3779B97F4A7C15ull;
    for (int i = 0; i < n; ++i)
        for (int j = 0; j < d; ++j) {
            x = x * 6364136223846793005ull + 1442695040888963407ull;
            const double u = (double)(x >> 11) * (1.0 / 9007199254740992.0);
            const bool bounded = (s->chain.bounded_mask >> j) & 1u;
            const double lo = bounded ? s->chain.qmin[j] : -3.0, hi = bounded ? s->chain.qmax[j] : 3.0;
            q[(size_t)i * d + j] = lo + (hi - lo) * u;
            seed[(size_t)i * d + j] = bounded ? 0.5 * (lo + hi) : 0.0;
        }
    if (int rc = pikamd_fk_batch(s, n, q.data(), goal.data())) return rc;
    struct Out {
        std::vector<double> sol, cost;
        std::vector<int32_t> st;
        std::vector<pikamd_stats> stats;
    };
    pik::SolverOptions saved = s->opt;
    auto run = [&](int lanes, bool passes, bool occ2, Out& o) -> int {
        s->opt = saved;
        s->opt.soa = false;
        s->opt.lpe = lanes;
        s->opt.n_sched = 0;
        s->opt.passes_set = true;
        s->opt.n_marks = 0;
        if (passes) {
            const int m[] = {1, 2, 3, 4, 7, 11, 16, 24, 40, 64};
            for (int v : m) s->opt.marks[s->opt.n_marks++] = v;
        }
        s->opt.two_per_simd = occ2 ? 1 : 0;
        s->opt.force_occ2 = occ2;
        s->opt.regime = 1;
        o.sol.assign((size_t)n * d, 0.0);
        o.cost.assign((size_t)n, 0.0);
        o.st.assign((size_t)n, 0);
        o.stats.assign((size_t)n, pikamd_stats{});
        const pikamd_batch b = {n,            goal.data(), seed.data(),   nullptr,        0,
                                o.sol.data(), o.st.data(), o.cost.data(), o.stats.data(), nullptr};
        int rc = start_job(s, p, 1, &b, 12345, pik::JOB_SELF_TEST);
        if (!rc) rc = wait_job(s, pik::JOB_SELF_TEST);
        s->opt = saved;
        return rc;
    };
    auto same = [&](const Out& a, const Out& b) {
        return std::memcmp(a.sol.data(), b.sol.data(), sizeof(double) * a.sol.size()) == 0 &&
               std::memcmp(a.cost.data(), b.cost.data(), sizeof(double) * a.cost.size()) == 0 &&
               std::memcmp(a.st.data(), b.st.data(), sizeof(int32_t) * a.st.size()) == 0 &&
               std::memcmp(a.stats.data(), b.stats.data(), sizeof(pikamd_stats) * a.stats.size()) == 0;
    };
    const bool multi = tips > 1;
    const int S = (p->mode == 0 && p->memetic_num_threads > 1) ? p->memetic_num_threads : 1;
    int gs = 1;
    while (p->mode == 0 && gs < p->memetic_elite_size) gs <<= 1;
    auto served = [&](int lanes) -> bool {
        if (mask_of(saved) & (unsigned)lanes) return false;
        return pik::lpe_allowed(s, lanes, gs, S, multi, exact_now);
    };
    Out ref, got;
    unsigned disabled = 0;
    if (p->mode != 0) {
        if (int rc = run(1, false, false, ref)) return rc;
#if !defined(PIK_STRICT)
        if (!needs_literal(s) && !exact_now)
            for (int lanes : {8, 16}) {
                if (!served(lanes)) continue;
                if (int rc = run(lanes, false, false, got)) return rc;
                if (!same(ref, got)) disabled |= (unsigned)lanes;
            }
#endif
        if (exact_now && !multi)
            for (int lanes : {4, 16}) {
                if (!served(lanes)) continue;
                if (int rc = run(lanes, false, false, got)) return rc;
                if (!same(ref, got)) disabled |= (unsigned)lanes;
            }
        mask_of(s->opt) = mask_of(saved) | disabled;
        if (disabled_out) *disabled_out = mask_of(s->opt);
        return 0;
    }
    if (int rc = run(1, false, false, ref)) return rc;
    for (int lanes : {2, 4, 8, 16}) {
        if (!served(lanes)) continue;
        for (int passes = 0; passes < 2; ++passes) {
            if (int rc = run(lanes, passes != 0, false, got)) return rc;
            if (!same(ref, got)) disabled |= (unsigned)lanes;
        }
    }
#if !defined(PIK_STRICT)
    {
        pik::ParamsK pk;
        if (!pik::make_params_k(p, pk) && common_eligible(s, p, pk)) {
            const bool was = s->opt.specialised;
            s->opt.specialised = false;
            Out general;
            saved.specialised = false;
            const int rc = run(1, false, false, general);
            saved.specialised = was;
            s->opt.specialised = was;
            if (rc) return rc;
            if (!same(ref, general)) disabled |= 32u;
        }
    }
#endif
    if (S == 1 && !multi) {
        if (int rc = run(1, false, true, got)) return rc;
        if (!same(ref, got)) disabled |= 1u;
    }
    if (int rc = run(1, true, false, got)) return rc;
    if (!same(ref, got)) return fail(PIKAMD_EHIP, "self test: the one-lane kernel disagrees with itself under compaction passes");
    if (disabled & 32u) s->opt.specialised = false;
    mask_of(s->opt) = mask_of(saved) | (disabled & ~32u);
    disabled = (disabled & 32u);
    if (disabled_out) *disabled_out = mask_of(s->opt) | disabled;
    return 0;
}

int32_t pikamd_self_test_cost(const pikamd_solver* s, int32_t* runs, double* total_ms) {
    if (!s) return fail(PIKAMD_EINVAL, "solver is NULL");
    if (runs) *runs = s->self_test_runs;
    if (total_ms) *total_ms = s->self_test_ms;
    return 0;
}

}

static int maybe_self_test(pikamd_solver* s, const pikamd_params* p) {
    if (!s->opt.auto_self_test || s->in_self_test || !p) return 0;
    pik::ParamsK pk;
    if (pik::make_params_k(p, pk)) return 0;
#if !defined(PIK_STRICT)
    if (common_eligible(s, p, pk) && common_ops(s->chain.dof, pk.goal_mask != 0)) return 0;
#endif
    unsigned long long h = 1469598103934665603ull;
    const long long key[] = {needs_literal(s, p) ? 1 : 0, p->mode, p->mode == 0 ? p->memetic_num_threads : 1,
                             p->mode == 0 ? p->memetic_elite_size : 0, pk.goal_mask, pk.line_delta, pk.approx,
                             pk.has_pos_thr, pk.has_ori_thr, pk.stop_on_valid, pk.stop_on_first,
                             p->position_scale > 0.0 ? 1 : 0, p->rotation_scale > 0.0 ? 1 : 0};
    const unsigned char* b = reinterpret_cast<const unsigned char*>(key);
    for (size_t i = 0; i < sizeof key; ++i) h = (h ^ b[i]) * 1099511628211ull;
    for (unsigned long long k : s->self_tested)
        if (k == h) return 0;
    pikamd_params q = *p;
    if (q.mode == 0) {
        q.memetic_max_generations = q.memetic_max_generations < 4 ? q.memetic_max_generations : 4;
        q.memetic_gd_max_iters = q.memetic_gd_max_iters < 6 ? q.memetic_gd_max_iters : 6;
    } else {
        q.gd_max_iters = q.gd_max_iters < 24 ? q.gd_max_iters : 24;
    }
    const auto t0 = std::chrono::steady_clock::now();
    s->in_self_test = true;
    const int rc = pikamd_self_test(s, &q, 32, nullptr);
    s->in_self_test = false;
    if (rc) return rc;
    s->self_test_runs += 1;
    s->self_test_ms += std::chrono::duration<double, std::milli>(std::chrono::steady_clock::now() - t0).count();
    s->self_tested.push_back(h);
    return 0;
}

extern "C" {

const char* pikamd_kernel_name(const pikamd_solver* s, const pikamd_params* p) {
    if (!s || !p) return "";
    pikamd_solver* m = const_cast<pikamd_solver*>(s);
    const char* ns = "pik";
#if defined(PIK_STRICT)
    ns = "pik_strict";
#else
    pik::ParamsK pk;
    if (needs_literal(s, p)) ns = "pik_exact";
    else if (!pik::make_params_k(p, pk) && common_eligible(s, p, pk) && common_ops(s->chain.dof, pk.goal_mask != 0))
        ns = pk.goal_mask != 0 ? "pik_common_goals" : "pik_common";
#endif
    snprintf(m->kernel_name, sizeof m->kernel_name, "%s::%s<%d>", ns,
             p->mode == 1 ? "ik_gradient_kernel" : "memetic_kernel", s->chain.dof);
    return m->kernel_name;
}

}

namespace {

int check_paths(const pikamd_solver* s, const pikamd_params* p, int64_t P, int32_t W, bool any_null, pik::ParamsK& pk) {
    if (int rc = check_solver(s)) return rc;
    if (!p) return fail(PIKAMD_EINVAL, "params is NULL");
    if (p->mode != 1)
        return fail(PIKAMD_EINVAL, "pikamd_solve_paths: waypoint paths are solved in local mode (mode = 1), got mode %d",
                    (int)p->mode);
    if (W < 1 || P < 0)
        return fail(PIKAMD_EINVAL, "pikamd_solve_paths: %lld paths of %d waypoints: expected P >= 0 and W >= 1",
                    (long long)P, (int)W);
    if (s->opt.soa)
        return fail(PIKAMD_EINVAL, "joint_layout soa: not with pikamd_solve_paths (its arrays are [P][W][dof])");
    if (const char* msg = pik::make_params_k(p, pk)) return fail(PIKAMD_EINVAL, "%s", msg);
    if (P > 0 && any_null)
        return fail(PIKAMD_EINVAL, "pikamd_solve_paths: goal_pos_quat, start, solution and status must not be NULL");
    return 0;
}

const char* path_flavour(const pikamd_solver* s, const pikamd_params* p, bool* exact) {
#if defined(PIK_STRICT)
    (void)s;
    (void)p;
    *exact = true;
    return "pik_strict";
#else
    *exact = needs_literal(s, p);
    return *exact ? "pik_exact" : "pik";
#endif
}

}

extern "C" {

int32_t pikamd_solve_paths_device(pikamd_solver* s, const pikamd_params* p, int64_t P, int32_t W,
                                  const double* d_goal_pos_quat, const double* d_start, const double* d_max_joint_step,
                                  double* d_solution, int32_t* d_status, double* d_final_cost, pikamd_stats* d_stats,
                                  int32_t* d_reached, void* stream, int32_t slot) {
    pik::ParamsK pk;
    if (int rc = check_paths(s, p, P, W, !d_goal_pos_quat || !d_start || !d_solution || !d_status, pk)) return rc;
    if (slot < 0 || slot >= PIKAMD_MAX_SLOTS) return fail(PIKAMD_EINVAL, "slot out of range");
    if (P == 0) return 0;
    const pik::PathOps* ops = path_ops_of(s, p);
    if (!ops) return no_kernels(s->chain.dof);
    HIP_TRY(hipSetDevice(s->device));
    const pik::PathArgs a = {P, W, 0, d_goal_pos_quat, d_start, d_max_joint_step, d_solution, d_status,
                             d_final_cost, d_stats, d_reached};
    return ops->solve(s, pk, a, (hipStream_t)stream, slot);
}

int32_t pikamd_solve_paths(pikamd_solver* s, const pikamd_params* p, int64_t P, int32_t W, const double* goal_pos_quat,
                           const double* start, const double* max_joint_step, double* solution, int32_t* status,
                           double* final_cost, pikamd_stats* stats, int32_t* reached) {
    pik::ParamsK pk;
    if (int rc = check_paths(s, p, P, W, !goal_pos_quat || !start || !solution || !status, pk)) return rc;
    if (P == 0) return 0;
    if (int rc = maybe_self_test(s, p)) return rc;
    const pik::PathOps* ops = path_ops_of(s, p);
    if (!ops) return no_kernels(s->chain.dof);
    const int job = PIKAMD_MAX_HOST_JOBS - 1;
    pik::HostJob& J = s->jobs[job];
    if (J.pending) return fail(PIKAMD_EINVAL, "job %d is still in flight: call pikamd_wait first", job);
    HIP_TRY(hipSetDevice(s->device));
    if (!J.stream) HIP_TRY(hipStreamCreateWithFlags(&J.stream, hipStreamNonBlocking));
    const size_t d = (size_t)s->chain.dof, g7 = 7 * (size_t)s->n_tips, rows = (size_t)P * (size_t)W;
    const size_t off_goal = 0, off_start = off_goal + sizeof(double) * g7 * rows;
    const size_t off_step = off_start + sizeof(double) * d * (size_t)P;
    const size_t in_bytes = off_step + (max_joint_step ? sizeof(double) * d : 0);
    const size_t off_solution = in_bytes, off_cost = off_solution + sizeof(double) * d * rows;
    const size_t off_stats = off_cost + sizeof(double) * rows, off_status = off_stats + sizeof(pikamd_stats) * rows;
    const size_t off_reached = off_status + align8(sizeof(int32_t) * rows);
    const size_t total = off_reached + align8(sizeof(int32_t) * (size_t)P);
    if (int rc = J.dev.ensure(total)) return rc;
    if (int rc = J.host.ensure(total)) return rc;
    char* hb = (char*)J.host.p;
    char* db = (char*)J.dev.p;
    std::memcpy(hb + off_goal, goal_pos_quat, sizeof(double) * g7 * rows);
    std::memcpy(hb + off_start, start, sizeof(double) * d * (size_t)P);
    if (max_joint_step) std::memcpy(hb + off_step, max_joint_step, sizeof(double) * d);
    HIP_TRY(hipMemcpyAsync(db, hb, in_bytes, hipMemcpyHostToDevice, J.stream));
    const pik::PathArgs a = {P, W, 0, (const double*)(db + off_goal), (const double*)(db + off_start),
                             max_joint_step ? (const double*)(db + off_step) : nullptr, (double*)(db + off_solution),
                             (int*)(db + off_status), (double*)(db + off_cost), (void*)(db + off_stats),
                             (int*)(db + off_reached)};
    if (int rc = ops->solve(s, pk, a, J.stream, pik::N_DEVICE_SLOTS + job)) {
        (void)hipStreamSynchronize(J.stream);
        return rc;
    }
    {
        hipError_t e = hipMemcpyAsync(hb + in_bytes, db + in_bytes, total - in_bytes, hipMemcpyDeviceToHost, J.stream);
        const hipError_t e2 = hipStreamSynchronize(J.stream);
        if (e == hipSuccess) e = e2;
        if (e != hipSuccess) return fail(PIKAMD_EHIP, "pikamd_solve_paths: %s (its results are lost)", hipGetErrorString(e));
    }
    std::memcpy(solution, hb + off_solution, sizeof(double) * d * rows);
    std::memcpy(status, hb + off_status, sizeof(int32_t) * rows);
    if (final_cost) std::memcpy(final_cost, hb + off_cost, sizeof(double) * rows);
    if (stats) std::memcpy(stats, hb + off_stats, sizeof(pikamd_stats) * rows);
    if (reached) std::memcpy(reached, hb + off_reached, sizeof(int32_t) * (size_t)P);
    return 0;
}

const char* pikamd_path_kernel_name(const pikamd_solver* s, const pikamd_params* p, int64_t P) {
    if (!s || !p) return "";
    pikamd_solver* m = const_cast<pikamd_solver*>(s);
    bool exact = false;
    const char* ns = path_flavour(s, p, &exact);
    const int lanes = pik::path_lanes(s, P, exact), dof = s->chain.dof;
    if (lanes == 1)
        snprintf(m->kernel_name, sizeof m->kernel_name, "%s::ik_path_kernel<%d,%s>", ns, dof, s->n_tips > 1 ? "true" : "false");
    else if (exact)
        snprintf(m->kernel_name, sizeof m->kernel_name, "%s::ik_path_team_kernel<%d,%d>", ns, dof, lanes);
    else
        snprintf(m->kernel_name, sizeof m->kernel_name, "%s::ik_path_wide_kernel<%d,%d,%s>", ns, dof, lanes,
                 s->n_tips > 1 ? "true" : "false");
    return m->kernel_name;
}

}

namespace {

int check_search(const pikamd_solver* s, const pikamd_params* p, int64_t B, int32_t K, bool any_null, pik::ParamsK& pk) {
    if (int rc = check_solver(s)) return rc;
    if (!p) return fail(PIKAMD_EINVAL, "params is NULL");
    if (p->mode != 1)
        return fail(PIKAMD_EINVAL,
                    "pikamd_search_batch: restarts are served in local mode (mode = 1), got mode %d: a restart attempt of "
                    "the memetic kernels would have to start a first pass from a device-side list of the failed problems, "
                    "which their launch does not offer",
                    (int)p->mode);
    if (K < 1 || K > PIKAMD_MAX_ATTEMPTS)
        return fail(PIKAMD_EINVAL, "pikamd_search_batch: max_attempts %d: expected 1..%d", (int)K, PIKAMD_MAX_ATTEMPTS);
    if (B < 0) return fail(PIKAMD_EINVAL, "pikamd_search_batch: B = %lld: expected B >= 0", (long long)B);
    if (s->opt.soa)
        return fail(PIKAMD_EINVAL, "joint_layout soa: not with pikamd_search_batch (its arrays are [B][dof])");
    if (const char* msg = pik::make_params_k(p, pk)) return fail(PIKAMD_EINVAL, "%s", msg);
    if (B > 0 && any_null)
        return fail(PIKAMD_EINVAL, "pikamd_search_batch: goal_pos_quat, seed, solution and status must not be NULL");
    return 0;
}

pik::SearchPlan search_plan_of(const pikamd_solver* s, const pikamd_params* p, int64_t B, int32_t K) {
    bool exact = false;
    (void)path_flavour(s, p, &exact);
    return pik::search_plan(s, ext_of(s)->search_schedule, B, K, exact);
}

int plan_search(pikamd_solver* s, const pikamd_params* p, int slot, pik::SearchArgs& a, double* all_solution,
                int32_t* all_status) {
    const pik::SearchPlan plan = search_plan_of(s, p, a.B, a.K);
    a.parallel = plan.parallel ? 1 : 0;
    a.lanes = plan.lanes;
    a.every = (all_solution || all_status) ? 1 : 0;
    a.row_solution = all_solution;
    a.row_status = all_status;
    a.row_cost = nullptr;
    a.row_stats = nullptr;
    if (!plan.parallel) return 0;
    const size_t rows = (size_t)a.B * (size_t)a.K, d = (size_t)s->chain.dof;
    const size_t off_stats = 0, off_cost = off_stats + sizeof(pikamd_stats) * rows;
    const size_t off_solution = off_cost + sizeof(double) * rows;
    const size_t off_status = off_solution + (all_solution ? 0 : sizeof(double) * d * rows);
    const size_t total = off_status + (all_status ? 0 : align8(sizeof(int32_t) * rows));
    pik::DevBuf& buf = ext_of(s)->search_rows[slot];
    if (int rc = buf.ensure(total)) return rc;
    char* w = (char*)buf.p;
    a.row_stats = w + off_stats;
    a.row_cost = (double*)(w + off_cost);
    if (!all_solution) a.row_solution = (double*)(w + off_solution);
    if (!all_status) a.row_status = (int*)(w + off_status);
    return 0;
}

}

extern "C" {

int32_t pikamd_search_batch_device(pikamd_solver* s, const pikamd_params* p, int64_t B, const double* d_goal_pos_quat,
                                   const double* d_seed, const double* d_initial_guess, uint64_t rng_seed,
                                   int64_t problem_offset, int32_t max_attempts, double* d_solution, int32_t* d_status,
                                   double* d_final_cost, pikamd_stats* d_stats, int32_t* d_attempts,
                                   double* d_all_solution, int32_t* d_all_status, void* stream, int32_t slot) {
    pik::ParamsK pk;
    if (int rc = check_search(s, p, B, max_attempts, !d_goal_pos_quat || !d_seed || !d_solution || !d_status, pk)) return rc;
    if (slot < 0 || slot >= PIKAMD_MAX_SLOTS) return fail(PIKAMD_EINVAL, "slot out of range");
    if (B == 0) return 0;
    const pik::SearchOps* ops = search_ops_of(s, p);
    if (!ops) return no_kernels(s->chain.dof);
    HIP_TRY(hipSetDevice(s->device));
    pik::SearchArgs a = {};
    a.B = B;
    a.K = max_attempts;
    a.goal = d_goal_pos_quat;
    a.seed = d_seed;
    a.guess = d_initial_guess ? d_initial_guess : d_seed;
    a.rng_seed = rng_seed;
    a.problem_offset = problem_offset;
    a.solution = d_solution;
    a.status = d_status;
    a.cost = d_final_cost;
    a.stats = d_stats;
    a.attempts = d_attempts;
    if (int rc = plan_search(s, p, slot, a, d_all_solution, d_all_status)) return rc;
    return ops->solve(s, pk, a, (hipStream_t)stream, slot);
}

int32_t pikamd_search_batch(pikamd_solver* s, const pikamd_params* p, int64_t B, const double* goal_pos_quat,
                            const double* seed, const double* initial_guess, uint64_t rng_seed, int64_t problem_offset,
                            int32_t max_attempts, double* solution, int32_t* status, double* final_cost,
                            pikamd_stats* stats, int32_t* attempts, double* all_solution, int32_t* all_status) {
    pik::ParamsK pk;
    if (int rc = check_search(s, p, B, max_attempts, !goal_pos_quat || !seed || !solution || !status, pk)) return rc;
    if (B == 0) return 0;
    if (int rc = maybe_self_test(s, p)) return rc;
    const pik::SearchOps* ops = search_ops_of(s, p);
    if (!ops) return no_kernels(s->chain.dof);
    const int job = PIKAMD_MAX_HOST_JOBS - 1;
    pik::HostJob& J = s->jobs[job];
    if (J.pending) return fail(PIKAMD_EINVAL, "job %d is still in flight: call pikamd_wait first", job);
    HIP_TRY(hipSetDevice(s->device));
    if (!J.stream) HIP_TRY(hipStreamCreateWithFlags(&J.stream, hipStreamNonBlocking));
    const size_t d = (size_t)s->chain.dof, g7 = 7 * (size_t)s->n_tips, n = (size_t)B, rows = n * (size_t)max_attempts;
    const size_t off_goal = 0, off_seed = off_goal + sizeof(double) * g7 * n, off_guess = off_seed + sizeof(double) * d * n;
    const size_t in_bytes = off_guess + (initial_guess ? sizeof(double) * d * n : 0);
    const size_t off_solution = in_bytes, off_cost = off_solution + sizeof(double) * d * n;
    const size_t off_stats = off_cost + sizeof(double) * n, off_status = off_stats + sizeof(pikamd_stats) * n;
    const size_t off_attempts = off_status + align8(sizeof(int32_t) * n);
    const size_t off_all_solution = off_attempts + align8(sizeof(int32_t) * n);
    const size_t off_all_status = off_all_solution + (all_solution ? sizeof(double) * d * rows : 0);
    const size_t total = off_all_status + (all_status ? align8(sizeof(int32_t) * rows) : 0);
    if (int rc = J.dev.ensure(total)) return rc;
    if (int rc = J.host.ensure(total)) return rc;
    char* hb = (char*)J.host.p;
    char* db = (char*)J.dev.p;
    pik::SearchArgs a = {};
    a.B = B;
    a.K = max_attempts;
    a.goal = (const double*)(db + off_goal);
    a.seed = (const double*)(db + off_seed);
    a.guess = initial_guess ? (const double*)(db + off_guess) : a.seed;
    a.rng_seed = rng_seed;
    a.problem_offset = problem_offset;
    a.solution = (double*)(db + off_solution);
    a.status = (int*)(db + off_status);
    a.cost = (double*)(db + off_cost);
    a.stats = (void*)(db + off_stats);
    a.attempts = (int*)(db + off_attempts);
    const int slot = pik::N_DEVICE_SLOTS + job;
    if (int rc = plan_search(s, p, slot, a, all_solution ? (double*)(db + off_all_solution) : nullptr,
                             all_status ? (int32_t*)(db + off_all_status) : nullptr))
        return rc;
    std::memcpy(hb + off_goal, goal_pos_quat, sizeof(double) * g7 * n);
    std::memcpy(hb + off_seed, seed, sizeof(double) * d * n);
    if (initial_guess) std::memcpy(hb + off_guess, initial_guess, sizeof(double) * d * n);
    HIP_TRY(hipMemcpyAsync(db, hb, in_bytes, hipMemcpyHostToDevice, J.stream));
    if (int rc = ops->solve(s, pk, a, J.stream, slot)) {
        (void)hipStreamSynchronize(J.stream);
        return rc;
    }
    {
        hipError_t e = hipMemcpyAsync(hb + in_bytes, db + in_bytes, total - in_bytes, hipMemcpyDeviceToHost, J.stream);
        const hipError_t e2 = hipStreamSynchronize(J.stream);
        if (e == hipSuccess) e = e2;
        if (e != hipSuccess) return fail(PIKAMD_EHIP, "pikamd_search_batch: %s (its results are lost)", hipGetErrorString(e));
    }
    std::memcpy(solution, hb + off_solution, sizeof(double) * d * n);
    std::memcpy(status, hb + off_status, sizeof(int32_t) * n);
    if (final_cost) std::memcpy(final_cost, hb + off_cost, sizeof(double) * n);
    if (stats) std::memcpy(stats, hb + off_stats, sizeof(pikamd_stats) * n);
    if (attempts) std::memcpy(attempts, hb + off_attempts, sizeof(int32_t) * n);
    if (all_solution) std::memcpy(all_solution, hb + off_all_solution, sizeof(double) * d * rows);
    if (all_status) std::memcpy(all_status, hb + off_all_status, sizeof(int32_t) * rows);
    return 0;
}

const char* pikamd_search_kernel_name(const pikamd_solver* s, const pikamd_params* p, int64_t B, int32_t max_attempts,
                                      int32_t* attempts_in_flight) {
    if (attempts_in_flight) *attempts_in_flight = 0;
    if (!s || !p || B < 0 || max_attempts < 1 || max_attempts > PIKAMD_MAX_ATTEMPTS) return "";
    pikamd_solver* m = const_cast<pikamd_solver*>(s);
    bool exact = false;
    const char* ns = path_flavour(s, p, &exact);
    const pik::SearchPlan plan = search_plan_of(s, p, B, max_attempts);
    const int lanes = plan.lanes, dof = s->chain.dof;
    if (attempts_in_flight) *attempts_in_flight = plan.parallel ? max_attempts : 1;
    if (lanes == 1)
        snprintf(m->kernel_name, sizeof m->kernel_name, "%s::ik_search_kernel<%d,%s>", ns, dof, s->n_tips > 1 ? "true" : "false");
    else if (exact)
        snprintf(m->kernel_name, sizeof m->kernel_name, "%s::ik_search_team_kernel<%d,%d>", ns, dof, lanes);
    else
        snprintf(m->kernel_name, sizeof m->kernel_name, "%s::ik_search_wide_kernel<%d,%d,%s>", ns, dof, lanes,
                 s->n_tips > 1 ? "true" : "false");
    return m->kernel_name;
}

}
```

pick_ik_amd/solver.py:

```python
from __future__ import annotations

import ctypes as C
import os

import numpy as np

_HERE = os.path.dirname(os.path.abspath(__file__))
LIB_PATH = os.environ.get("PIK_LIB") or os.path.join(_HERE, "libpick_ik_amd.so")
LIB_STRICT_PATH = os.environ.get("PIK_LIB_STRICT") or os.path.join(_HERE, "libpick_ik_amd_strict.so")

SUCCESS = 1
APPROXIMATE = 2
NO_IK_SOLUTION = -31
NOT_ATTEMPTED = 0
PATH_JUMP = -1001
MAX_ATTEMPTS = 64
MAX_SLOTS = 128
MAX_BATCHES = 64
MAX_HOST_JOBS = 16


class PickIkAmdError(RuntimeError):
    pass


class Params(C.Structure):

    _fields_ = [
        ("mode", C.c_int32),
        ("gd_step_size", C.c_double),
        ("gd_max_iters", C.c_int32),
        ("gd_min_cost_delta", C.c_double),
        ("position_threshold", C.c_double),
        ("orientation_threshold", C.c_double),
        ("cost_threshold", C.c_double),
        ("position_scale", C.c_double),
        ("rotation_scale", C.c_double),
        ("center_joints_weight", C.c_double),
        ("avoid_joint_limits_weight", C.c_double),
        ("minimal_displacement_weight", C.c_double),
        ("stop_optimization_on_valid_solution", C.c_int32),
        ("memetic_num_threads", C.c_int32),
        ("memetic_stop_on_first_solution", C.c_int32),
        ("memetic_population_size", C.c_int32),
        ("memetic_elite_size", C.c_int32),
        ("memetic_wipeout_fitness_tol", C.c_double),
        ("memetic_max_generations", C.c_int32),
        ("memetic_gd_max_iters", C.c_int32),
        ("return_approximate_solution", C.c_int32),
    ]


class _Chain(C.Structure):
    _fields_ = [
        ("dof", C.c_int32),
        ("origin_xyz_rpy", C.POINTER(C.c_double)),
        ("axis", C.POINTER(C.c_double)),
        ("joint_type", C.POINTER(C.c_int32)),
        ("tip_xyz_rpy", C.POINTER(C.c_double)),
        ("qmin", C.POINTER(C.c_double)),
        ("qmax", C.POINTER(C.c_double)),
        ("vmax", C.POINTER(C.c_double)),
        ("bounded", C.POINTER(C.c_uint8)),
    ]


class _Tip(C.Structure):
    _fields_ = [
        ("n_joints", C.c_int32),
        ("variable", C.POINTER(C.c_int32)),
        ("origin_xyz_rpy", C.POINTER(C.c_double)),
        ("axis", C.POINTER(C.c_double)),
        ("joint_type", C.POINTER(C.c_int32)),
        ("tip_xyz_rpy", C.POINTER(C.c_double)),
    ]


class _MultiChain(C.Structure):
    _fields_ = [
        ("dof", C.c_int32),
        ("n_tips", C.c_int32),
        ("tips", C.POINTER(_Tip)),
        ("qmin", C.POINTER(C.c_double)),
        ("qmax", C.POINTER(C.c_double)),
        ("vmax", C.POINTER(C.c_double)),
        ("bounded", C.POINTER(C.c_uint8)),
    ]


class Batch(C.Structure):

    _fields_ = [
        ("B", C.c_int64),
        ("goal_pos_quat", C.c_void_p),
        ("seed", C.c_void_p),
        ("initial_guess", C.c_void_p),
        ("problem_offset", C.c_int64),
        ("solution", C.c_void_p),
        ("status", C.c_void_p),
        ("final_cost", C.c_void_p),
        ("stats", C.c_void_p),
        ("completed", C.c_void_p),
    ]


MAX_DOF, MAX_TIPS, MAX_NAME, MAX_MIMIC = 16, 8, 64, 4


class _UrdfTip(C.Structure):
    _fields_ = [("n_joints", C.c_int32), ("variable", C.c_int32 * MAX_DOF),
                ("origin_xyz_rpy", C.c_double * 6 * MAX_DOF), ("axis", C.c_double * 3 * MAX_DOF),
                ("joint_type", C.c_int32 * MAX_DOF), ("tip_xyz_rpy", C.c_double * 6)]


class MimicJointC(C.Structure):
    _fields_ = [("tip", C.c_int32), ("after_variable", C.c_int32), ("master_variable", C.c_int32), ("joint_type", C.c_int32),
                ("origin_xyz_rpy", C.c_double * 6), ("axis", C.c_double * 3), ("multiplier", C.c_double), ("offset", C.c_double)]


def mimic_array(chain):
    ms = tuple(getattr(chain, "mimic", ()) or ())
    if not ms:
        return None
    arr = (MimicJointC * len(ms))()
    for i, m in enumerate(ms):
        arr[i] = MimicJointC(int(m.tip), int(m.after_variable), int(m.master_variable), int(m.joint_type),
                             (C.c_double * 6)(*[float(x) for x in m.origin_xyz_rpy]), (C.c_double * 3)(*[float(x) for x in m.axis]),
                             float(m.multiplier), float(m.offset))
    return arr


class UrdfModel(C.Structure):

    _fields_ = [("dof", C.c_int32), ("n_tips", C.c_int32), ("variable_names", (C.c_char * MAX_NAME) * MAX_DOF),
                ("qmin", C.c_double * MAX_DOF), ("qmax", C.c_double * MAX_DOF), ("vmax", C.c_double * MAX_DOF),
                ("bounded", C.c_uint8 * MAX_DOF), ("tips", _UrdfTip * MAX_TIPS),
                ("n_mimic", C.c_int32), ("mimic", MimicJointC * (MAX_TIPS * MAX_MIMIC))]


STATS_DTYPE = np.dtype(
    [("cost_evals", "<i8"), ("generations", "<i4"), ("wipeouts", "<i4"),
     ("pool_erasures", "<i4"), ("reserved", "<i4")])

EXPORTED_SYMBOLS = (
    "pikamd_default_params", "pikamd_create", "pikamd_destroy", "pikamd_variables",
    "pikamd_fk_batch", "pikamd_cost_batch", "pikamd_gd_step_batch", "pikamd_solve_batch",
    "pikamd_solve_batch_device", "pikamd_fk_batch_device", "pikamd_last_error", "pikamd_version",
    "pikamd_kernel_name", "pikamd_reserve", "pikamd_create_multi", "pikamd_n_tips",
    "pikamd_solve_batches_device", "pikamd_solve_batches_async", "pikamd_wait", "pikamd_solve_batches",
    "pikamd_urdf_extract", "pikamd_create_from_urdf", "pikamd_set_option", "pikamd_solve_batch_host", "pikamd_set_mimic_joints",
    "pikamd_shard_bounds", "pikamd_solve_batch_sharded", "pikamd_self_test", "pikamd_self_test_cost",
    "pikamd_solve_paths", "pikamd_solve_paths_device", "pikamd_path_kernel_name",
    "pikamd_search_batch", "pikamd_search_batch_device", "pikamd_search_kernel_name",
)

_libs = {}


COST_FN = C.CFUNCTYPE(C.c_double, C.POINTER(C.c_double), C.c_int32, C.c_int32, C.c_void_p)


def cost_callback(fn):
    def trampoline(q, dof, pose, _user):
        return float(fn(np.ctypeslib.as_array(q, shape=(dof,)).copy(), int(pose)))
    return COST_FN(trampoline)


def lib(strict: bool = False):
    if strict in _libs:
        return _libs[strict]
    path = LIB_STRICT_PATH if strict else LIB_PATH
    if not os.path.exists(path):
        raise PickIkAmdError(
            f"{path} is missing: build it with `python -c 'import __graft_entry__ as g; "
            "g.build()'` (hipcc --offload-arch=gfx950). pick_ik_amd has no CPU fallback.")
    L = C.CDLL(path)
    dp = C.POINTER(C.c_double)
    ip = C.POINTER(C.c_int32)
    vp = C.c_void_p
    L.pikamd_default_params.argtypes = [C.POINTER(Params)]
    L.pikamd_default_params.restype = None
    L.pikamd_create.argtypes = [C.POINTER(_Chain), C.c_int32, C.POINTER(vp)]
    L.pikamd_create_multi.argtypes = [C.POINTER(_MultiChain), C.c_int32, C.POINTER(vp)]
    L.pikamd_create_multi.restype = C.c_int32
    L.pikamd_n_tips.argtypes = [vp]
    L.pikamd_n_tips.restype = C.c_int32
    L.pikamd_destroy.argtypes = [vp]
    L.pikamd_destroy.restype = None
    L.pikamd_variables.argtypes = [vp, dp]
    L.pikamd_fk_batch.argtypes = [vp, C.c_int64, dp, dp]
    L.pikamd_cost_batch.argtypes = [vp, C.POINTER(Params), C.c_int64, dp, dp, dp, dp, ip]
    L.pikamd_gd_step_batch.argtypes = [vp, C.POINTER(Params), C.c_int64, dp, dp, dp, dp, dp, dp,
                                       dp, ip]
    L.pikamd_solve_batch.argtypes = [vp, C.POINTER(Params), C.c_int64, dp, dp, C.c_uint64,
                                     C.c_int64, dp, ip, dp, vp]
    L.pikamd_solve_batch_device.argtypes = [vp, C.POINTER(Params), C.c_int64, vp, vp, C.c_uint64,
                                            C.c_int64, vp, vp, vp, vp, vp, C.c_int32]
    L.pikamd_fk_batch_device.argtypes = [vp, C.c_int64, vp, vp, vp]
    L.pikamd_solve_batches_device.argtypes = [vp, C.POINTER(Params), C.c_int32, C.POINTER(Batch),
                                              C.c_uint64, vp, C.c_int32]
    L.pikamd_solve_batches_async.argtypes = [vp, C.POINTER(Params), C.c_int32, C.POINTER(Batch),
                                             C.c_uint64, C.c_int32]
    L.pikamd_wait.argtypes = [vp, C.c_int32]
    L.pikamd_solve_batches.argtypes = [vp, C.POINTER(Params), C.c_int32, C.POINTER(Batch), C.c_uint64]
    L.pikamd_reserve.argtypes = [vp, C.POINTER(Params), C.c_int64, C.c_int32, vp]
    L.pikamd_reserve.restype = C.c_int32
    L.pikamd_urdf_extract.argtypes = [C.c_char_p, C.c_char_p, C.POINTER(C.c_char_p), C.c_int32,
                                      C.POINTER(UrdfModel)]
    L.pikamd_urdf_extract.restype = C.c_int32
    L.pikamd_create_from_urdf.argtypes = [C.c_char_p, C.c_char_p, C.POINTER(C.c_char_p), C.c_int32, C.c_int32,
                                          C.POINTER(vp)]
    L.pikamd_create_from_urdf.restype = C.c_int32
    L.pikamd_shard_bounds.argtypes = [C.c_int64, C.c_int32, C.c_int32, C.POINTER(C.c_int64), C.POINTER(C.c_int64)]
    L.pikamd_shard_bounds.restype = None
    L.pikamd_solve_batch_sharded.argtypes = [C.POINTER(vp), C.c_int32, C.POINTER(Params), C.c_int64, dp, dp, dp,
                                             C.c_uint64, C.c_int64, dp, ip, dp, vp]
    L.pikamd_solve_batch_sharded.restype = C.c_int32
    L.pikamd_self_test.argtypes = [vp, C.POINTER(Params), C.c_int32, C.POINTER(C.c_uint32)]
    L.pikamd_self_test.restype = C.c_int32
    L.pikamd_self_test_cost.argtypes = [vp, C.POINTER(C.c_int32), C.POINTER(C.c_double)]
    L.pikamd_self_test_cost.restype = C.c_int32
    L.pikamd_set_option.argtypes = [vp, C.c_char_p, C.c_char_p]
    L.pikamd_set_option.restype = C.c_int32
    L.pikamd_solve_batch_host.argtypes = [vp, C.POINTER(Params), C.c_int64, dp, dp, dp, C.c_uint64, C.c_int64, COST_FN,
                                          vp, dp, ip, dp, vp]
    L.pikamd_solve_batch_host.restype = C.c_int32
    L.pikamd_set_mimic_joints.argtypes = [vp, C.c_int32, C.POINTER(MimicJointC)]
    L.pikamd_set_mimic_joints.restype = C.c_int32
    L.pikamd_last_error.restype = C.c_char_p
    L.pikamd_version.restype = C.c_char_p
    L.pikamd_kernel_name.restype = C.c_char_p
    L.pikamd_kernel_name.argtypes = [vp, C.POINTER(Params)]
    L.pikamd_solve_paths.argtypes = [vp, C.POINTER(Params), C.c_int64, C.c_int32, dp, dp, dp, dp, ip, dp, vp, ip]
    L.pikamd_solve_paths.restype = C.c_int32
    L.pikamd_solve_paths_device.argtypes = [vp, C.POINTER(Params), C.c_int64, C.c_int32, vp, vp, vp, vp, vp, vp, vp, vp,
                                            vp, C.c_int32]
    L.pikamd_solve_paths_device.restype = C.c_int32
    L.pikamd_path_kernel_name.argtypes = [vp, C.POINTER(Params), C.c_int64]
    L.pikamd_path_kernel_name.restype = C.c_char_p
    L.pikamd_search_batch.argtypes = [vp, C.POINTER(Params), C.c_int64, dp, dp, dp, C.c_uint64, C.c_int64, C.c_int32,
                                      dp, ip, dp, vp, ip, dp, ip]
    L.pikamd_search_batch.restype = C.c_int32
    L.pikamd_search_batch_device.argtypes = [vp, C.POINTER(Params), C.c_int64, vp, vp, vp, C.c_uint64, C.c_int64,
                                             C.c_int32, vp, vp, vp, vp, vp, vp, vp, vp, C.c_int32]
    L.pikamd_search_batch_device.restype = C.c_int32
    L.pikamd_search_kernel_name.argtypes = [vp, C.POINTER(Params), C.c_int64, C.c_int32, ip]
    L.pikamd_search_kernel_name.restype = C.c_char_p
    for name in ("pikamd_create", "pikamd_variables", "pikamd_fk_batch", "pikamd_cost_batch",
                 "pikamd_gd_step_batch", "pikamd_solve_batch", "pikamd_solve_batch_device",
                 "pikamd_fk_batch_device", "pikamd_solve_batches_device",
                 "pikamd_solve_batches_async", "pikamd_wait", "pikamd_solve_batches"):
        getattr(L, name).restype = C.c_int32
    _libs[strict] = L
    return L


def _check(rc: int, L=None):
    if rc != 0:
        L = L or lib()
        raise PickIkAmdError(f"pick_ik_amd error {rc}: {L.pikamd_last_error().decode()}")


def default_params(**kw) -> Params:
    p = Params()
    lib().pikamd_default_params(C.byref(p))
    for k, v in kw.items():
        if not hasattr(p, k):
            raise AttributeError(k)
        setattr(p, k, v)
    return p


def _f64(a):
    return np.ascontiguousarray(a, dtype=np.float64)


def _dp(a):
    return a.ctypes.data_as(C.POINTER(C.c_double))


def _ip(a):
    return a.ctypes.data_as(C.POINTER(C.c_int32))


def _urdf_text(urdf: str) -> bytes:
    text = urdf if urdf.lstrip().startswith("<") else open(urdf).read()
    return text.encode()


def urdf_extract(urdf: str, base_link: str, tip_links, strict: bool = False):
    from .robots import Chain, multi_chain
    L = lib(strict)
    tips = [tip_links] if isinstance(tip_links, str) else list(tip_links)
    arr = (C.c_char_p * len(tips))(*[t.encode() for t in tips])
    m = UrdfModel()
    _check(L.pikamd_urdf_extract(_urdf_text(urdf), base_link.encode(), arr, len(tips), C.byref(m)), L)
    d = m.dof
    names = [m.variable_names[i].value.decode() for i in range(d)]
    lim = [np.array(m.qmin[:d]), np.array(m.qmax[:d]), np.array(m.vmax[:d]), np.array(m.bounded[:d], dtype=np.uint8)]

    def tip_arrays(t):
        n = t.n_joints
        return (list(t.variable[:n]), np.array([list(r) for r in t.origin_xyz_rpy[:n]]).reshape(n, 6),
                np.array([list(r) for r in t.axis[:n]]).reshape(n, 3), np.array(t.joint_type[:n], dtype=np.int32),
                np.array(t.tip_xyz_rpy[:]))

    from .robots import MimicJoint
    import dataclasses
    mim = tuple(MimicJoint(after_variable=x.after_variable, master_variable=x.master_variable,
                           origin_xyz_rpy=tuple(x.origin_xyz_rpy), axis=tuple(x.axis), multiplier=x.multiplier,
                           offset=x.offset, joint_type=x.joint_type, tip=x.tip) for x in m.mimic[:m.n_mimic])
    if m.n_tips == 1:
        _, o, a, jt, tip = tip_arrays(m.tips[0])
        return Chain(name="urdf", origin_xyz_rpy=o, axis=a, joint_type=jt, tip_xyz_rpy=tip, qmin=lim[0],
                     qmax=lim[1], vmax=lim[2], bounded=lim[3], mimic=mim), names
    paths = [tip_arrays(m.tips[k]) for k in range(m.n_tips)]
    mc = multi_chain("urdf", paths, *lim)
    return (dataclasses.replace(mc, mimic=mim) if mim else mc), names


class Solver:

    def __init__(self, chain, device: int = 0, strict: bool = False, exact=None):
        self._L = lib(strict)
        self.strict = strict
        self.exact = (exact is None or bool(exact)) and not strict
        self.chain = chain
        self.dof = int(chain.dof)
        self.device = int(device)
        self.n_tips = int(getattr(chain, "n_tips", 1))
        h = C.c_void_p()
        lim = [_f64(chain.qmin), _f64(chain.qmax), _f64(chain.vmax),
               np.ascontiguousarray(chain.bounded, dtype=np.uint8)]
        if hasattr(chain, "tips"):
            keep, tips = [lim], (_Tip * self.n_tips)()
            for i, t in enumerate(chain.tips):
                a = [np.ascontiguousarray(t.variable, dtype=np.int32), _f64(t.origin_xyz_rpy),
                     _f64(t.axis), np.ascontiguousarray(t.joint_type, dtype=np.int32),
                     _f64(t.tip_xyz_rpy)]
                keep.append(a)
                tips[i] = _Tip(len(a[0]), _ip(a[0]), _dp(a[1]), _dp(a[2]), _ip(a[3]), _dp(a[4]))
            self._keep = (keep, tips)
            c = _MultiChain(self.dof, self.n_tips, tips, _dp(lim[0]), _dp(lim[1]), _dp(lim[2]),
                            lim[3].ctypes.data_as(C.POINTER(C.c_uint8)))
            self._chk(self._L.pikamd_create_multi(C.byref(c), self.device, C.byref(h)))
        else:
            k = [_f64(chain.origin_xyz_rpy), _f64(chain.axis),
                 np.ascontiguousarray(chain.joint_type, dtype=np.int32), _f64(chain.tip_xyz_rpy)]
            self._keep = (k, lim)
            c = _Chain(self.dof, _dp(k[0]), _dp(k[1]), _ip(k[2]), _dp(k[3]), _dp(lim[0]),
                       _dp(lim[1]), _dp(lim[2]), lim[3].ctypes.data_as(C.POINTER(C.c_uint8)))
            self._chk(self._L.pikamd_create(C.byref(c), self.device, C.byref(h)))
        self._h = h
        arr = mimic_array(chain)
        if arr is not None:
            self._chk(self._L.pikamd_set_mimic_joints(self._h, len(arr), arr))
        if not self.strict and exact is not None:
            self.set_option("arithmetic", "exact" if exact else "fast")
        self._env_options()

    @classmethod
    def from_urdf(cls, urdf: str, base_link: str, tip_links, device: int = 0, strict: bool = False):
        chain, names = urdf_extract(urdf, base_link, tip_links, strict)
        self = cls.__new__(cls)
        self._L = lib(strict)
        self.strict, self.chain, self.variable_names = strict, chain, names
        self.exact = not strict
        self.dof, self.device, self.n_tips = int(chain.dof), int(device), int(getattr(chain, "n_tips", 1))
        tips = [tip_links] if isinstance(tip_links, str) else list(tip_links)
        arr = (C.c_char_p * len(tips))(*[t.encode() for t in tips])
        h = C.c_void_p()
        self._keep = None
        _check(self._L.pikamd_create_from_urdf(_urdf_text(urdf), base_link.encode(), arr, len(tips), self.device,
                                               C.byref(h)), self._L)
        self._h = h
        return self

    def _chk(self, rc: int):
        _check(rc, self._L)

    def set_option(self, name: str, value) -> None:
        v = b"" if value is None else str(value).encode()
        self._chk(self._L.pikamd_set_option(self._h, name.encode(), v))

    def self_test(self, params: Params, n: int = 64) -> int:
        m = C.c_uint32(0)
        self._chk(self._L.pikamd_self_test(self._h, C.byref(params), n, C.byref(m)))
        return int(m.value)

    def self_test_cost(self):
        runs, ms = C.c_int32(0), C.c_double(0.0)
        self._chk(self._L.pikamd_self_test_cost(self._h, C.byref(runs), C.byref(ms)))
        return int(runs.value), float(ms.value)

    ENV_OPTIONS = (("PIK_LPE", "lanes_per_elite"), ("PIK_LPE_SCHED", "lanes_per_elite_schedule"),
                   ("PIK_PASSES", "passes"), ("PIK_OCC2", "two_per_simd"), ("PIK_REGIME", "regime"),
                   ("PIK_SPECIALISED", "specialised"), ("PIK_SHARD_CHUNKS", "shard_chunks"),
                   ("PIK_SELF_TEST", "self_test"))

    def _env_options(self) -> None:
        cur = tuple(os.environ.get(k) for k, _ in self.ENV_OPTIONS)
        seen = getattr(self, "_env_seen", (None,) * len(cur))
        if cur == seen:
            return
        for (_, name), new, old in zip(self.ENV_OPTIONS, cur, seen):
            if new != old:
                self.set_option(name, new)
        self._env_seen = cur

    def close(self):
        if getattr(self, "_h", None):
            self._L.pikamd_destroy(self._h)
            self._h = None

    def __del__(self):
        try:
            self.close()
        except Exception:
            pass

    def variables(self) -> np.ndarray:
        out = np.empty((self.dof, 7))
        self._chk(self._L.pikamd_variables(self._h, _dp(out)))
        return out

    def fk(self, q) -> np.ndarray:
        q = _f64(q).reshape(-1, self.dof)
        out = np.empty((q.shape[0], 7) if self.n_tips == 1 else (q.shape[0], self.n_tips, 7))
        self._chk(self._L.pikamd_fk_batch(self._h, q.shape[0], _dp(q), _dp(out)))
        return out

    def cost(self, params: Params, goal_pos_quat, seed, q):
        q = _f64(q).reshape(-1, self.dof)
        n = q.shape[0]
        g7 = 7 * self.n_tips
        goal = np.ascontiguousarray(np.broadcast_to(_f64(goal_pos_quat).reshape(-1, g7), (n, g7)))
        seed = np.ascontiguousarray(np.broadcast_to(_f64(seed).reshape(-1, self.dof),
                                                    (n, self.dof)))
        cost = np.empty(n)
        sol = np.empty(n, dtype=np.int32)
        self._chk(self._L.pikamd_cost_batch(self._h, C.byref(params), n, _dp(goal), _dp(seed), _dp(q),
                                       _dp(cost), _ip(sol)))
        return cost, sol

    def gd_step(self, params: Params, goal_pos_quat, seed, local, best, local_cost, best_cost):
        local = _f64(local).reshape(-1, self.dof).copy()
        n = local.shape[0]
        best = _f64(best).reshape(n, self.dof).copy()
        goal = _f64(goal_pos_quat).reshape(n, 7 * self.n_tips)
        seed = _f64(seed).reshape(n, self.dof)
        lc = _f64(local_cost).reshape(n).copy()
        bc = _f64(best_cost).reshape(n).copy()
        grad = np.empty((n, self.dof))
        imp = np.empty(n, dtype=np.int32)
        self._chk(self._L.pikamd_gd_step_batch(self._h, C.byref(params), n, _dp(goal), _dp(seed),
                                          _dp(local), _dp(best), _dp(lc), _dp(bc), _dp(grad),
                                          _ip(imp)))
        return local, best, lc, bc, grad, imp

    def _host_batch(self, goal_pos_quat, seed, initial_guess=None, problem_offset=0):
        goal = _f64(goal_pos_quat).reshape(-1, 7 * self.n_tips)
        B = goal.shape[0]
        seed = _f64(seed).reshape(B, self.dof)
        guess = None if initial_guess is None else _f64(initial_guess).reshape(B, self.dof)
        sol = np.empty((B, self.dof))
        status = np.empty(B, dtype=np.int32)
        cost = np.empty(B)
        stats = np.zeros(B, dtype=STATS_DTYPE)
        b = Batch(B, goal.ctypes.data, seed.ctypes.data, None if guess is None else guess.ctypes.data,
                  problem_offset, sol.ctypes.data, status.ctypes.data, cost.ctypes.data,
                  stats.ctypes.data, None)
        return b, (goal, seed, guess), (sol, status, cost, stats)

    def solve_batch(self, params: Params, goal_pos_quat, seed, rng_seed: int = 0,
                    problem_offset: int = 0, initial_guess=None):
        self._env_options()
        if initial_guess is None:
            goal = _f64(goal_pos_quat).reshape(-1, 7 * self.n_tips)
            B = goal.shape[0]
            seed = _f64(seed).reshape(B, self.dof)
            sol = np.empty((B, self.dof))
            status = np.empty(B, dtype=np.int32)
            cost = np.empty(B)
            stats = np.zeros(B, dtype=STATS_DTYPE)
            self._chk(self._L.pikamd_solve_batch(self._h, C.byref(params), B, _dp(goal), _dp(seed),
                                                 C.c_uint64(rng_seed), problem_offset, _dp(sol),
                                                 _ip(status), _dp(cost),
                                                 stats.ctypes.data_as(C.c_void_p)))
            return sol, status, cost, stats
        return self.solve_batches(params, [(goal_pos_quat, seed, initial_guess, problem_offset)],
                                  rng_seed=rng_seed)[0]

    def solve_batch_host(self, params: Params, goal_pos_quat, seed, cost_fn, rng_seed: int = 0, problem_offset: int = 0,
                         initial_guess=None):
        goal = _f64(goal_pos_quat).reshape(-1, 7 * self.n_tips)
        B = goal.shape[0]
        seed = _f64(seed).reshape(B, self.dof)
        guess = None if initial_guess is None else _f64(initial_guess).reshape(B, self.dof)
        sol = np.empty((B, self.dof))
        status = np.empty(B, dtype=np.int32)
        cost = np.empty(B)
        stats = np.zeros(B, dtype=STATS_DTYPE)
        cb = cost_fn if isinstance(cost_fn, COST_FN) else cost_callback(cost_fn)
        self._chk(self._L.pikamd_solve_batch_host(self._h, C.byref(params), B, _dp(goal), _dp(seed),
                                                  None if guess is None else _dp(guess), C.c_uint64(rng_seed),
                                                  problem_offset, cb, None, _dp(sol), _ip(status), _dp(cost),
                                                  stats.ctypes.data_as(C.c_void_p)))
        return sol, status, cost, stats

    def solve_batches(self, params: Params, batches, rng_seed: int = 0, job: int | None = None):
        self._env_options()
        made = [self._host_batch(g, sd, ig, off) for g, sd, ig, off in batches]
        arr = (Batch * len(made))(*[m[0] for m in made])
        if job is None:
            self._chk(self._L.pikamd_solve_batches(self._h, C.byref(params), len(made), arr,
                                                   C.c_uint64(rng_seed)))
        else:
            self._chk(self._L.pikamd_solve_batches_async(self._h, C.byref(params), len(made), arr,
                                                         C.c_uint64(rng_seed), job))
            self._jobs = getattr(self, "_jobs", {})
            self._jobs[job] = made
        return [m[2] for m in made]

    def wait(self, job: int):
        self._chk(self._L.pikamd_wait(self._h, job))
        getattr(self, "_jobs", {}).pop(job, None)

    def solve_batch_device(self, params: Params, B: int, d_goal: int, d_seed: int, d_solution: int,
                           d_status: int, d_cost: int = 0, d_stats: int = 0, rng_seed: int = 0,
                           problem_offset: int = 0, stream: int = 0, slot: int = 0):
        self._env_options()
        self._chk(self._L.pikamd_solve_batch_device(
            self._h, C.byref(params), B, d_goal, d_seed, C.c_uint64(rng_seed), problem_offset,
            d_solution, d_status, d_cost or None, d_stats or None, stream or None, slot))

    def solve_batches_device(self, params: Params, batches, rng_seed: int = 0, stream: int = 0,
                             slot: int = 0):
        self._env_options()
        arr = (Batch * len(batches))(*[b if isinstance(b, Batch) else Batch(**b) for b in batches])
        self._chk(self._L.pikamd_solve_batches_device(self._h, C.byref(params), len(batches), arr,
                                                      C.c_uint64(rng_seed), stream or None, slot))

    def reserve(self, params: Params, B: int, slot: int = 0, stream: int = 0):
        self._env_options()
        self._chk(self._L.pikamd_reserve(self._h, C.byref(params), B, slot, stream or None))

    def fk_device(self, n: int, d_q: int, d_pos_quat: int, stream: int = 0):
        self._chk(self._L.pikamd_fk_batch_device(self._h, n, d_q, d_pos_quat, stream or None))

    def kernel_name(self, params: Params) -> str:
        return self._L.pikamd_kernel_name(self._h, C.byref(params)).decode()

    def solve_paths(self, params: Params, goals, start, max_joint_step=None):
        self._env_options()
        goals = _f64(goals)
        tail = (7,) if self.n_tips == 1 else (self.n_tips, 7)
        if goals.ndim != 2 + len(tail) or goals.shape[2:] != tail:
            raise ValueError(f"goals: expected [P][W]{list(tail)}, got {list(goals.shape)}")
        P, W = goals.shape[:2]
        if W < 1:
            raise ValueError("goals: a path has at least one waypoint")
        start = _f64(start)
        if start.shape != (P, self.dof):
            raise ValueError(f"start: expected [{P}][{self.dof}], got {list(start.shape)}")
        step = None
        if max_joint_step is not None:
            step = _f64(max_joint_step)
            if step.shape != (self.dof,):
                raise ValueError(f"max_joint_step: expected [{self.dof}], got {list(step.shape)}")
        sol = np.empty((P, W, self.dof))
        status = np.empty((P, W), dtype=np.int32)
        cost = np.empty((P, W))
        stats = np.zeros((P, W), dtype=STATS_DTYPE)
        reached = np.empty(P, dtype=np.int32)
        self._chk(self._L.pikamd_solve_paths(self._h, C.byref(params), P, W, _dp(goals), _dp(start),
                                             None if step is None else _dp(step), _dp(sol), _ip(status), _dp(cost),
                                             stats.ctypes.data_as(C.c_void_p), _ip(reached)))
        return sol, status, cost, stats, reached

    def solve_paths_device(self, params: Params, P: int, W: int, d_goals: int, d_start: int, d_solution: int,
                           d_status: int, d_max_joint_step: int = 0, d_cost: int = 0, d_stats: int = 0,
                           d_reached: int = 0, stream: int = 0, slot: int = 0):
        self._env_options()
        if P < 0 or W < 1:
            raise ValueError(f"{P} paths of {W} waypoints: expected P >= 0 and W >= 1")
        self._chk(self._L.pikamd_solve_paths_device(
            self._h, C.byref(params), P, W, d_goals or None, d_start or None, d_max_joint_step or None,
            d_solution or None, d_status or None, d_cost or None, d_stats or None, d_reached or None, stream or None,
            slot))

    def path_kernel_name(self, params: Params, P: int) -> str:
        self._env_options()
        return self._L.pikamd_path_kernel_name(self._h, C.byref(params), P).decode()

    def search_batch(self, params: Params, goal_pos_quat, seed, max_attempts: int, rng_seed: int = 0,
                     problem_offset: int = 0, initial_guess=None, all_attempts: bool = False):
        self._env_options()
        goal = _f64(goal_pos_quat)
        if goal.ndim < 2 or goal.size != goal.shape[0] * 7 * self.n_tips:
            raise ValueError(f"goal_pos_quat: expected [B]{[7] if self.n_tips == 1 else [self.n_tips, 7]}, "
                             f"got {list(goal.shape)}")
        B = goal.shape[0]
        seed = _f64(seed)
        if seed.shape != (B, self.dof):
            raise ValueError(f"seed: expected [{B}][{self.dof}], got {list(seed.shape)}")
        guess = None
        if initial_guess is not None:
            guess = _f64(initial_guess)
            if guess.shape != (B, self.dof):
                raise ValueError(f"initial_guess: expected [{B}][{self.dof}], got {list(guess.shape)}")
        K = int(max_attempts)
        if not 1 <= K <= MAX_ATTEMPTS:
            raise ValueError(f"max_attempts: expected 1..{MAX_ATTEMPTS}, got {max_attempts}")
        sol = np.empty((B, self.dof))
        status = np.empty(B, dtype=np.int32)
        cost = np.empty(B)
        stats = np.zeros(B, dtype=STATS_DTYPE)
        attempts = np.empty(B, dtype=np.int32)
        all_sol = np.empty((B, K, self.dof)) if all_attempts else None
        all_st = np.empty((B, K), dtype=np.int32) if all_attempts else None
        self._chk(self._L.pikamd_search_batch(
            self._h, C.byref(params), B, _dp(goal), _dp(seed), None if guess is None else _dp(guess),
            C.c_uint64(rng_seed), problem_offset, K, _dp(sol), _ip(status), _dp(cost), stats.ctypes.data_as(C.c_void_p),
            _ip(attempts), None if all_sol is None else _dp(all_sol), None if all_st is None else _ip(all_st)))
        if all_attempts:
            return sol, status, cost, stats, attempts, all_sol, all_st
        return sol, status, cost, stats, attempts

    def search_batch_device(self, params: Params, B: int, d_goal: int, d_seed: int, max_attempts: int, d_solution: int,
                            d_status: int, d_initial_guess: int = 0, d_cost: int = 0, d_stats: int = 0,
                            d_attempts: int = 0, d_all_solution: int = 0, d_all_status: int = 0, rng_seed: int = 0,
                            problem_offset: int = 0, stream: int = 0, slot: int = 0):
        self._env_options()
        self._chk(self._L.pikamd_search_batch_device(
            self._h, C.byref(params), B, d_goal or None, d_seed or None, d_initial_guess or None, C.c_uint64(rng_seed),
            problem_offset, max_attempts, d_solution or None, d_status or None, d_cost or None, d_stats or None,
            d_attempts or None, d_all_solution or None, d_all_status or None, stream or None, slot))

    def search_kernel_name(self, params: Params, B: int, max_attempts: int):
        self._env_options()
        n = C.c_int32(0)
        name = self._L.pikamd_search_kernel_name(self._h, C.byref(params), B, max_attempts, C.byref(n)).decode()
        return name, int(n.value)


def shard_bounds(total: int, rank: int, world: int, strict: bool = False):
    lo, hi = C.c_int64(), C.c_int64()
    lib(strict).pikamd_shard_bounds(total, rank, world, C.byref(lo), C.byref(hi))
    return lo.value, hi.value


def solve_batch_sharded(solvers, params: Params, goal_pos_quat, seed, rng_seed: int = 0, problem_offset: int = 0,
                        initial_guess=None):
    s0 = solvers[0]
    for s in solvers:
        s._env_options()
    goal = _f64(goal_pos_quat).reshape(-1, 7 * s0.n_tips)
    B = goal.shape[0]
    seed = _f64(seed).reshape(B, s0.dof)
    guess = None if initial_guess is None else _f64(initial_guess).reshape(B, s0.dof)
    sol = np.empty((B, s0.dof))
    status = np.empty(B, dtype=np.int32)
    cost = np.empty(B)
    stats = np.zeros(B, dtype=STATS_DTYPE)
    arr = (C.c_void_p * len(solvers))(*[s._h for s in solvers])
    _check(s0._L.pikamd_solve_batch_sharded(arr, len(solvers), C.byref(params), B, _dp(goal), _dp(seed),
                                            None if guess is None else _dp(guess), C.c_uint64(rng_seed),
                                            problem_offset, _dp(sol), _ip(status), _dp(cost),
                                            stats.ctypes.data_as(C.c_void_p)), s0._L)
    return sol, status, cost, stats


def ik_memetic(solver: Solver, initial_guess, goal_pos_quat, params: Params | None = None,
               approx_solution: bool = False, rng_seed: int = 0):
    p = params or default_params()
    p.mode = 0
    p.return_approximate_solution = int(approx_solution)
    sol, status, _, _ = solver.solve_batch(p, goal_pos_quat, initial_guess, rng_seed=rng_seed)
    return sol, status > 0


def ik_gradient(solver: Solver, initial_guess, goal_pos_quat, params: Params | None = None,
                approx_solution: bool = False):
    p = params or default_params()
    p.mode = 1
    p.return_approximate_solution = int(approx_solution)
    sol, status, _, _ = solver.solve_batch(p, goal_pos_quat, initial_guess)
    return sol, status > 0
```

Baseline: 2.819 million solves/s.

## Route memetic solve passes to kernel variants on device using cross-stream load

```diff
diff --git a/include/pick_ik_amd.h b/include/pick_ik_amd.h
--- a/include/pick_ik_amd.h
+++ b/include/pick_ik_amd.h
@@ -240,6 +240,8 @@
                                    double* d_all_solution, int32_t* d_all_status, void* stream, int32_t slot);
 const char* pikamd_search_kernel_name(const pikamd_solver* s, const pikamd_params* p, int64_t B,
                                       int32_t max_attempts, int32_t* attempts_in_flight);
+int32_t pikamd_debug_regime(pikamd_solver* s, int32_t slot, int64_t publish_load, int32_t max_passes,
+                            int32_t* n_passes, uint32_t* survivors, uint32_t* others_load, int32_t* variant);
 
 #ifdef __cplusplus
 }
diff --git a/pick_ik_amd/build.py b/pick_ik_amd/build.py
--- a/pick_ik_amd/build.py
+++ b/pick_ik_amd/build.py
@@ -12,7 +12,7 @@
 LIB = os.path.join(_HERE, "libpick_ik_amd.so")
 LIB_STRICT = os.path.join(_HERE, "libpick_ik_amd_strict.so")
 HEADERS = ["pik_kernels.hpp", "pik_math.hpp", "pik_host.hpp", "pik_solver.hpp", "pik_launch.hpp", "pik_exact.hpp",
-           "pik_host_solve.hpp", "pik_path.hpp", "pik_path_ops.hpp", "pik_search.hpp", "pik_search_ops.hpp"]
+           "pik_host_solve.hpp", "pik_path.hpp", "pik_path_ops.hpp", "pik_search.hpp", "pik_search_ops.hpp", "pik_route.hpp", "pik_route_ops.hpp"]
 HEADER = os.path.join(os.path.dirname(_HERE), "include", "pick_ik_amd.h")
 DOFS = tuple(range(1, 17))
 BUILD_DIR = os.path.join(_HERE, "_build")
@@ -82,6 +82,22 @@
     keep = {int(x) for x in only.split(",")} if only else set(DOFS)
     return [(os.path.join(d, f"pik_search_inst_d{n}.o"), "pik_search_inst.hip",
              [f"-DPIK_INST_D={n}"] + (fl if n in keep else ["-DPIK_INST_STUB=1"] + fl)) for n in DOFS]
+
+
+ROUTE_FLAVOURS = ("fast", "exact", "common", "common_goals")
+
+
+def _route_objects(flavour: str):
+    d = os.path.join(BUILD_DIR, flavour)
+    fl = {"fast": [], "exact": EXACT_FLAGS, "common": COMMON_FLAGS, "common_goals": COMMON_GOALS_FLAGS}[flavour]
+    only = os.environ.get("PIK_ONLY_D")
+    keep = {int(x) for x in only.split(",")} if only else set(DOFS)
+    return [(os.path.join(d, f"pik_route_inst_d{n}.o"), "pik_route_inst.hip",
+             [f"-DPIK_INST_D={n}"] + (fl if n in keep else ["-DPIK_INST_STUB=1"] + fl)) for n in DOFS]
+
+
+def _all_route_objects():
+    return [o for fl in ROUTE_FLAVOURS for o in _route_objects(fl)]
 
 
 def _common_objects(goals: bool = False):
@@ -174,14 +190,14 @@
 
 
 def _sources():
-    return ([os.path.join(CSRC, f) for f in ("pik_amd.hip", "pik_inst.hip", "pik_path_inst.hip", "pik_search_inst.hip", "pik_urdf.hpp",
+    return ([os.path.join(CSRC, f) for f in ("pik_amd.hip", "pik_inst.hip", "pik_path_inst.hip", "pik_search_inst.hip", "pik_route_inst.hip", "pik_urdf.hpp",
                                              *HEADERS)] +
             [HEADER, os.path.abspath(__file__)])
 
 
 def _lib_stamp(strict: bool) -> str:
     flags = _flavor_flags(strict) + ([] if strict else ["+exact:"] + EXACT_FLAGS + ["+common:"] + COMMON_FLAGS + ["+common_goals:"] + COMMON_GOALS_FLAGS)
-    return _stamp(flags + ["+paths", "+search", "only=" + os.environ.get("PIK_ONLY_D", "all")])
+    return _stamp(flags + ["+paths", "+search"] + ([] if strict else ["+route"]) + ["only=" + os.environ.get("PIK_ONLY_D", "all")])
 
 
 def is_stale(lib: str = LIB) -> bool:
@@ -277,9 +293,9 @@
     rows = []
     for o in (_objects(False) + _exact_objects() + _common_objects() + _common_objects(True) + _objects(True) +
               _path_objects("fast") + _path_objects("exact") + _path_objects("strict") +
-              _search_objects("fast") + _search_objects("exact") + _search_objects("strict")):
+              _search_objects("fast") + _search_objects("exact") + _search_objects("strict") + _all_route_objects()):
         res = o[0] + ".res"
-        if o[1] not in ("pik_inst.hip", "pik_path_inst.hip", "pik_search_inst.hip"):
+        if o[1] not in ("pik_inst.hip", "pik_path_inst.hip", "pik_search_inst.hip", "pik_route_inst.hip"):
             continue
         if not os.path.exists(res):
             return None
@@ -321,6 +337,8 @@
             objs = objs + _exact_objects() + _common_objects() + _common_objects(True)
         objs = objs + (_path_objects("strict") if strict else _path_objects("fast") + _path_objects("exact"))
         objs = objs + (_search_objects("strict") if strict else _search_objects("fast") + _search_objects("exact"))
+        if not strict:
+            objs = objs + _all_route_objects()
         stale = [o for o in objs if force or _obj_stale(*o, _is_strict_obj(o))]
         jobs += [(o, _is_strict_obj(o)) for o in stale if (o, _is_strict_obj(o)) not in jobs]
         relink.append((lib, [o[0] for o in objs]))
diff --git a/pick_ik_amd/csrc/pik_amd.hip b/pick_ik_amd/csrc/pik_amd.hip
--- a/pick_ik_amd/csrc/pik_amd.hip
+++ b/pick_ik_amd/csrc/pik_amd.hip
@@ -10,6 +10,7 @@
 #include <vector>
 
 #include "pik_path_ops.hpp"
+#include "pik_route_ops.hpp"
 #include "pik_search_ops.hpp"
 #include "pik_solver.hpp"
 #include "pik_urdf.hpp"
@@ -43,6 +44,12 @@
 PIK_LITERAL_SEARCH_OPS(9) PIK_LITERAL_SEARCH_OPS(10) PIK_LITERAL_SEARCH_OPS(11) PIK_LITERAL_SEARCH_OPS(12)
 PIK_LITERAL_SEARCH_OPS(13) PIK_LITERAL_SEARCH_OPS(14) PIK_LITERAL_SEARCH_OPS(15) PIK_LITERAL_SEARCH_OPS(16)
 #undef PIK_LITERAL_SEARCH_OPS
+#define PIK_FLAVOUR_ROUTE_OPS(N) const void* route_ops_d##N();
+PIK_FLAVOUR_ROUTE_OPS(1) PIK_FLAVOUR_ROUTE_OPS(2) PIK_FLAVOUR_ROUTE_OPS(3) PIK_FLAVOUR_ROUTE_OPS(4)
+PIK_FLAVOUR_ROUTE_OPS(5) PIK_FLAVOUR_ROUTE_OPS(6) PIK_FLAVOUR_ROUTE_OPS(7) PIK_FLAVOUR_ROUTE_OPS(8)
+PIK_FLAVOUR_ROUTE_OPS(9) PIK_FLAVOUR_ROUTE_OPS(10) PIK_FLAVOUR_ROUTE_OPS(11) PIK_FLAVOUR_ROUTE_OPS(12)
+PIK_FLAVOUR_ROUTE_OPS(13) PIK_FLAVOUR_ROUTE_OPS(14) PIK_FLAVOUR_ROUTE_OPS(15) PIK_FLAVOUR_ROUTE_OPS(16)
+#undef PIK_FLAVOUR_ROUTE_OPS
 }
 namespace pik_common {
 char* error_buffer() { return ::pik::error_buffer(); }
@@ -51,6 +58,12 @@
 PIK_COMMON_OPS(7) PIK_COMMON_OPS(8) PIK_COMMON_OPS(9) PIK_COMMON_OPS(10) PIK_COMMON_OPS(11) PIK_COMMON_OPS(12)
 PIK_COMMON_OPS(13) PIK_COMMON_OPS(14) PIK_COMMON_OPS(15) PIK_COMMON_OPS(16)
 #undef PIK_COMMON_OPS
+#define PIK_FLAVOUR_ROUTE_OPS(N) const void* route_ops_d##N();
+PIK_FLAVOUR_ROUTE_OPS(1) PIK_FLAVOUR_ROUTE_OPS(2) PIK_FLAVOUR_ROUTE_OPS(3) PIK_FLAVOUR_ROUTE_OPS(4)
+PIK_FLAVOUR_ROUTE_OPS(5) PIK_FLAVOUR_ROUTE_OPS(6) PIK_FLAVOUR_ROUTE_OPS(7) PIK_FLAVOUR_ROUTE_OPS(8)
+PIK_FLAVOUR_ROUTE_OPS(9) PIK_FLAVOUR_ROUTE_OPS(10) PIK_FLAVOUR_ROUTE_OPS(11) PIK_FLAVOUR_ROUTE_OPS(12)
+PIK_FLAVOUR_ROUTE_OPS(13) PIK_FLAVOUR_ROUTE_OPS(14) PIK_FLAVOUR_ROUTE_OPS(15) PIK_FLAVOUR_ROUTE_OPS(16)
+#undef PIK_FLAVOUR_ROUTE_OPS
 }
 namespace pik_common_goals {
 char* error_buffer() { return ::pik::error_buffer(); }
@@ -59,6 +72,12 @@
 PIK_COMMON_OPS(7) PIK_COMMON_OPS(8) PIK_COMMON_OPS(9) PIK_COMMON_OPS(10) PIK_COMMON_OPS(11) PIK_COMMON_OPS(12)
 PIK_COMMON_OPS(13) PIK_COMMON_OPS(14) PIK_COMMON_OPS(15) PIK_COMMON_OPS(16)
 #undef PIK_COMMON_OPS
+#define PIK_FLAVOUR_ROUTE_OPS(N) const void* route_ops_d##N();
+PIK_FLAVOUR_ROUTE_OPS(1) PIK_FLAVOUR_ROUTE_OPS(2) PIK_FLAVOUR_ROUTE_OPS(3) PIK_FLAVOUR_ROUTE_OPS(4)
+PIK_FLAVOUR_ROUTE_OPS(5) PIK_FLAVOUR_ROUTE_OPS(6) PIK_FLAVOUR_ROUTE_OPS(7) PIK_FLAVOUR_ROUTE_OPS(8)
+PIK_FLAVOUR_ROUTE_OPS(9) PIK_FLAVOUR_ROUTE_OPS(10) PIK_FLAVOUR_ROUTE_OPS(11) PIK_FLAVOUR_ROUTE_OPS(12)
+PIK_FLAVOUR_ROUTE_OPS(13) PIK_FLAVOUR_ROUTE_OPS(14) PIK_FLAVOUR_ROUTE_OPS(15) PIK_FLAVOUR_ROUTE_OPS(16)
+#undef PIK_FLAVOUR_ROUTE_OPS
 }
 #endif
 
@@ -67,6 +86,12 @@
 struct SolverExt : pikamd_solver {
     int search_schedule = pik::SEARCH_ADAPTIVE;
     pik::DevBuf search_rows[pik::N_SLOTS];
+    int device_regime = 1;
+    long long regime_threshold = 0;
+    int routed_passes[pik::N_SLOTS];
+    SolverExt() {
+        for (int& v : routed_passes) v = -1;
+    }
 };
 SolverExt* ext_of(pikamd_solver* s) { return static_cast<SolverExt*>(s); }
 const SolverExt* ext_of(const pikamd_solver* s) { return static_cast<const SolverExt*>(s); }
@@ -146,6 +171,49 @@
     (void)pk;
 #endif
     return ops_of(s, p);
+}
+
+[[maybe_unused]] const pik::RouteOps* route_ops_of(const pikamd_solver* s, const pikamd_params* p, const pik::ParamsK& pk) {
+#if !defined(PIK_STRICT)
+    const pik::SolverOptions& o = s->opt;
+    if (!ext_of(s)->device_regime || p->mode != 0 || s->n_tips != 1 || p->memetic_num_threads > 1 || o.lpe != 0 ||
+        o.n_sched != 0 || o.regime != 0)
+        return nullptr;
+    const bool common = common_eligible(s, p, pk), goals = pk.goal_mask != 0, literal = needs_literal(s, p);
+    const void* r = nullptr;
+    switch (s->chain.dof) {
+#define PIK_ROUTE_CASE(N)                                                                                             \
+    case N:                                                                                                           \
+        r = common ? (goals ? pik_common_goals::route_ops_d##N() : pik_common::route_ops_d##N())                      \
+                   : literal ? pik_exact::route_ops_d##N() : static_cast<const void*>(pik::route_ops_d##N());         \
+        break;
+        PIK_ROUTE_CASE(1) PIK_ROUTE_CASE(2) PIK_ROUTE_CASE(3) PIK_ROUTE_CASE(4) PIK_ROUTE_CASE(5) PIK_ROUTE_CASE(6)
+        PIK_ROUTE_CASE(7) PIK_ROUTE_CASE(8) PIK_ROUTE_CASE(9) PIK_ROUTE_CASE(10) PIK_ROUTE_CASE(11) PIK_ROUTE_CASE(12)
+        PIK_ROUTE_CASE(13) PIK_ROUTE_CASE(14) PIK_ROUTE_CASE(15) PIK_ROUTE_CASE(16)
+#undef PIK_ROUTE_CASE
+        default: break;
+    }
+    return static_cast<const pik::RouteOps*>(r);
+#else
+    (void)s, (void)p, (void)pk;
+    return nullptr;
+#endif
+}
+
+int run_solve(pikamd_solver* s, const pikamd_params* p, const pik::ParamsK& pk, pik::BatchRecord* rec, int n,
+              unsigned long long rng_seed, hipStream_t stream, int slot) {
+    SolverExt* x = ext_of(s);
+    if (const pik::RouteOps* r = route_ops_of(s, p, pk)) {
+        pik::RouteCtx ctx;
+        ctx.threshold = x->regime_threshold;
+        if (int rc = r->solve(s, p, pk, rec, n, rng_seed, stream, slot, &ctx)) return rc;
+        if (ctx.served) {
+            x->routed_passes[slot] = ctx.n_passes;
+            return 0;
+        }
+    }
+    x->routed_passes[slot] = -1;
+    return solve_ops_of(s, p, pk)->solve(s, p, pk, rec, n, rng_seed, stream, slot, false);
 }
 
 int no_kernels(int dof) {
@@ -248,8 +316,8 @@
     s->n_tips = n_tips;
     for (int k = 1; k < n_tips; ++k) s->more[k - 1] = chains[k];
     const size_t table_bytes = sizeof(pik::BatchRecord) * PIKAMD_MAX_BATCHES * pik::TABLE_RING;
-    hipError_t e = hipMalloc(reinterpret_cast<void**>(&s->counters), pik::COUNTER_BLOCK * pik::N_SLOTS);
-    if (e == hipSuccess) e = hipMemset(s->counters, 0, pik::COUNTER_BLOCK * pik::N_SLOTS);
+    hipError_t e = hipMalloc(reinterpret_cast<void**>(&s->counters), pik::COUNTERS_BYTES);
+    if (e == hipSuccess) e = hipMemset(s->counters, 0, pik::COUNTERS_BYTES);
     if (e == hipSuccess) e = hipMalloc(reinterpret_cast<void**>(&s->consts_dev), pik::CONSTS_STRIDE * pik::N_SLOTS);
     if (e == hipSuccess)
         e = hipHostMalloc(reinterpret_cast<void**>(&s->consts_host), pik::CONSTS_STRIDE * pik::N_SLOTS, hipHostMallocDefault);
@@ -557,7 +625,7 @@
     if (const char* msg = pik::make_params_k(p, pk)) return fail(PIKAMD_EINVAL, "%s", msg);
     if (n == 0) return 0;
     HIP_TRY(hipSetDevice(s->device));
-    if (!s->opt.soa) return solve_ops_of(s, p, pk)->solve(s, p, pk, rec, n, rng_seed, stream, slot, false);
+    if (!s->opt.soa) return run_solve(s, p, pk, rec, n, rng_seed, stream, slot);
     const int D = s->chain.dof;
     size_t doubles = 0;
     for (int k = 0; k < n; ++k) {
@@ -594,7 +662,7 @@
         rec[k].solution = w;
         w += (size_t)B * D;
     }
-    if (int rc = solve_ops_of(s, p, pk)->solve(s, p, pk, rec, n, rng_seed, stream, slot, false)) return rc;
+    if (int rc = run_solve(s, p, pk, rec, n, rng_seed, stream, slot)) return rc;
     for (int k = 0; k < n; ++k)
         if (int rc = move(rec[k].solution, user_solution[k], rec[k].B, 0)) return rc;
     return 0;
@@ -901,6 +969,21 @@
         if (v == "sequential") { sched = pik::SEARCH_SEQUENTIAL; return 0; }
         if (v == "parallel") { sched = pik::SEARCH_PARALLEL; return 0; }
         return fail(PIKAMD_EINVAL, "search_schedule: expected 'adaptive', 'sequential' or 'parallel', got '%s'", v.c_str());
+    }
+    if (n == "device_regime") {
+        int x = 1;
+        if (!pik::parse_device_regime(v.c_str(), &x))
+            return fail(PIKAMD_EINVAL, "device_regime: expected '0' or '1', got '%s'", v.c_str());
+        ext_of(s)->device_regime = x;
+        return 0;
+    }
+    if (n == "regime_threshold") {
+        if (v.empty()) { ext_of(s)->regime_threshold = 0; return 0; }
+        std::vector<int> x;
+        if (!ints(v, ',', x) || x.size() != 1 || x[0] < 0)
+            return fail(PIKAMD_EINVAL, "regime_threshold: expected a number of problems >= 0, got '%s'", v.c_str());
+        ext_of(s)->regime_threshold = x[0];
+        return 0;
     }
     if (n == "regime") {
         if (v.empty() || v == "adaptive") { o.regime = 0; return 0; }
@@ -1504,4 +1587,31 @@
     return m->kernel_name;
 }
 
-}
+
+int32_t pikamd_debug_regime(pikamd_solver* s, int32_t slot, int64_t publish_load, int32_t max_passes,
+                            int32_t* n_passes, uint32_t* survivors, uint32_t* others_load, int32_t* variant) {
+    if (int rc = check_solver(s)) return rc;
+    if (slot < 0 || slot >= pik::N_SLOTS) return fail(PIKAMD_EINVAL, "slot out of range");
+    if (max_passes < 0 || (max_passes > 0 && (!survivors || !others_load || !variant)))
+        return fail(PIKAMD_EINVAL, "bad arguments");
+    HIP_TRY(hipSetDevice(s->device));
+    HIP_TRY(hipDeviceSynchronize());
+    if (publish_load >= 0) {
+        const uint32_t v = publish_load > 0xffffffffll ? 0xffffffffu : (uint32_t)publish_load;
+        HIP_TRY(hipMemcpy(pik::route_loads(s) + slot, &v, sizeof v, hipMemcpyHostToDevice));
+    }
+    const int routed = ext_of(s)->routed_passes[slot];
+    if (n_passes) *n_passes = routed;
+    if (routed > 0 && max_passes > 0) {
+        uint32_t rec[pik::ROUTE_MAX_PASSES * 4];
+        HIP_TRY(hipMemcpy(rec, pik::route_record(s, slot), sizeof rec, hipMemcpyDeviceToHost));
+        for (int k = 0; k < routed && k < max_passes; ++k) {
+            survivors[k] = rec[4 * k + 0];
+            others_load[k] = rec[4 * k + 1];
+            variant[k] = (int32_t)rec[4 * k + 2];
+        }
+    }
+    return 0;
+}
+
+}
diff --git a/pick_ik_amd/csrc/pik_route.hpp b/pick_ik_amd/csrc/pik_route.hpp
--- /dev/null
+++ b/pick_ik_amd/csrc/pik_route.hpp
@@ -0,0 +1,288 @@
+#pragma once
+
+#include "pik_launch.hpp"
+#include "pik_route_ops.hpp"
+
+namespace pik {
+
+struct RouteTable {
+    int n;
+    int var[ROUTE_MAX_VARIANTS];
+    int id[ROUTE_MAX_VARIANTS];
+    unsigned hi[ROUTE_MAX_VARIANTS];
+};
+
+struct RouteArgs {
+    unsigned* count;
+    unsigned fixed_n;
+    int fixed_id;
+    unsigned* vc;
+    unsigned* loads;
+    unsigned* record;
+    int slot, n_slots;
+    int clear;
+    unsigned long long threshold;
+    RouteTable lat, thr;
+};
+
+template <int D>
+__global__ __launch_bounds__(WAVE) void route_kernel(RouteArgs r) {
+    __shared__ unsigned long long part[WAVE];
+    const int lane = threadIdx.x;
+    unsigned long long mine = 0ull;
+    for (int i = lane; i < r.n_slots; i += WAVE)
+        if (i != r.slot) mine += __hip_atomic_load(r.loads + i, __ATOMIC_RELAXED, __HIP_MEMORY_SCOPE_AGENT);
+    part[lane] = mine;
+    __syncthreads();
+    if (lane != 0) return;
+    if (r.clear) {
+        __hip_atomic_store(r.loads + r.slot, 0u, __ATOMIC_RELAXED, __HIP_MEMORY_SCOPE_AGENT);
+        return;
+    }
+    unsigned long long others = 0ull;
+    for (int i = 0; i < WAVE; ++i) others += part[i];
+    const unsigned n = r.count ? *r.count : r.fixed_n;
+    __hip_atomic_store(r.loads + r.slot, n, __ATOMIC_RELAXED, __HIP_MEMORY_SCOPE_AGENT);
+    int id = r.fixed_id;
+    if (r.count) {
+        const RouteTable& t = (others >= r.threshold) ? r.thr : r.lat;
+        int pick = -1;
+        for (int i = 0; i < t.n; ++i)
+            if (pick < 0 && n > 0u && n <= t.hi[i]) pick = i;
+        id = 0;
+        if (pick >= 0) {
+            r.vc[t.var[pick]] = n;
+            id = t.id[pick];
+        }
+        *r.count = 0u;
+    }
+    if (r.record) {
+        r.record[0] = n;
+        r.record[1] = others > 0xffffffffull ? 0xffffffffu : (unsigned)others;
+        r.record[2] = (unsigned)id;
+        r.record[3] = 1u;
+    }
+}
+
+template <int D>
+int launch_solve_routed(pikamd_solver* s, const pikamd_params* p, const ParamsK& pk, BatchRecord* batches,
+                        int n_batches, unsigned long long rng_seed, hipStream_t st, int slot, RouteCtx* ctx) {
+    ctx->served = false;
+    ctx->n_passes = 0;
+    long long B = 0;
+    for (int k = 0; k < n_batches; ++k) B += batches[k].B;
+    if (B == 0 || p->mode != 0 || s->n_tips != 1 || p->memetic_num_threads > 1) return 0;
+    SolveArgs a;
+    std::memset(&a, 0, sizeof a);
+    a.gs_log2 = pow2ceil_log2(pk.elites);
+    const int gs = 1 << a.gs_log2;
+    const int S = 1;
+    a.species = S;
+    a.sp_log2 = 0;
+    Schedule sc;
+    make_schedule(s, pk, gs, S, sc);
+    if (sc.n_sched > 0 || s->opt.regime != 0) return 0;
+    bool host_throughput = false;
+    {
+        int others = 0;
+        for (int k = 0; k < N_DEVICE_SLOTS + N_HOST_JOBS; ++k)
+            if (k != slot && s->slot_event_used[k] && hipEventQuery(s->slot_event[k]) == hipErrorNotReady) ++others;
+        (void)hipGetLastError();
+        host_throughput = others >= 3;
+    }
+    const long long occ2_from_thr = sc.occ2_from;
+    const long long occ2_from_lat =
+        (s->opt.two_per_simd < 2 && !s->opt.force_occ2) ? (long long)s->num_cu * 4 * 9 / 8 : sc.occ2_from;
+    int n_marks = sc.n_marks;
+    if (!host_throughput && !s->opt.passes_set) {
+        int widest = 1;
+        for (int l : {16, 8, 4, 2})
+            if (widest == 1 && lpe_allowed(s, l, gs, S, false)) widest = l;
+        if (widest > 1 && B <= (long long)s->num_cu * 4 * (WAVE / (gs * widest))) n_marks = 0;
+    }
+    if (n_marks == 0) return 0;
+    static_assert(sizeof(Schedule::marks) / sizeof(int) <= ROUTE_MAX_PASSES, "a record per pass");
+
+    const ConstsK<D>* kc = nullptr;
+    if (int rc = upload_consts<D>(s, &pk, slot, st, &kc)) return rc;
+    TableSlot table;
+    a.n_batches = n_batches;
+    for (int k = 0; k < n_batches; ++k) a.signal |= batches[k].completed != nullptr;
+    a.rng_seed = rng_seed;
+    a.B = B;
+    const long long cap = B;
+    const size_t recs = (size_t)B * (size_t)S;
+    const size_t d_rows = (size_t)StateRows<D>::D_ROWS(pk.elites);
+    const size_t off_d = 0;
+    const size_t off_l = off_d + sizeof(double) * d_rows * recs;
+    const size_t off_i = off_l + sizeof(long long) * StateRows<D>::L_ROWS * recs;
+    const size_t off_list = off_i + sizeof(int) * StateRows<D>::I_ROWS * recs;
+    const size_t off_cnt = off_list + sizeof(int) * 2 * (size_t)cap;
+    const bool has_unbounded = s->chain.bounded_mask != ((1u << s->chain.dof) - 1u);
+    const size_t pop_stride = (size_t)pk.population * (1 + D) + ((size_t)pk.population + 1) / 2;
+    const size_t off_pop = (off_cnt + 64 + 63) / 64 * 64;
+    const size_t total = off_pop + (has_unbounded ? sizeof(double) * 2 * pop_stride * (size_t)cap * (size_t)S : 0);
+    if (int rc = s->slot_state[slot].ensure(total)) return rc;
+    if (int rc = upload_batch_table(s, batches, n_batches, st, &a.batches, &a.B, table)) return rc;
+    char* base = (char*)s->slot_state[slot].p;
+    a.pop = has_unbounded ? (double*)(base + off_pop) : nullptr;
+    a.pop_stride = (long long)pop_stride;
+    a.cap = cap;
+    a.st_d = (double*)(base + off_d);
+    a.st_l = (long long*)(base + off_l);
+    a.st_i = (int*)(base + off_i);
+    int* lists[2] = {(int*)(base + off_list), (int*)(base + off_list) + cap};
+    unsigned char* cblk = s->counters + COUNTER_BLOCK * (size_t)slot;
+    unsigned long long* c_work = (unsigned long long*)cblk;
+    unsigned* c_nlist = (unsigned*)(cblk + 128);
+    unsigned* c_done = (unsigned*)(cblk + 256);
+    unsigned* vc = route_vc(s, slot);
+    if (s->counters_dirty[slot]) {
+        HIP_TRY(hipMemsetAsync(cblk, 0, COUNTER_BLOCK, st));
+        HIP_TRY(hipMemsetAsync(vc, 0, ROUTE_VC_BLOCK, st));
+    }
+    s->counters_dirty[slot] = true;
+
+    auto capacity_of = [&](auto kernel, int variant, long long* cap_out) -> int {
+        int per_cu = s->occupancy_cache[PIK_OCC_ROW][variant];
+        if (per_cu == 0) {
+            HIP_TRY(hipOccupancyMaxActiveBlocksPerMultiprocessor(&per_cu, kernel, WAVE, 0));
+            if (per_cu < 1) per_cu = 1;
+            s->occupancy_cache[PIK_OCC_ROW][variant] = per_cu;
+        }
+        *cap_out = (long long)s->num_cu * per_cu;
+        return 0;
+    };
+    struct Variant {
+        int lpe, id;
+        long long capacity;
+    };
+    Variant var[ROUTE_MAX_VARIANTS];
+    int n_var = 0;
+    auto add_variant = [&](auto kernel, int lpe_, int id) -> int {
+        Variant v{lpe_, id, 0};
+        if (int rc = capacity_of(kernel, id, &v.capacity)) return rc;
+        var[n_var++] = v;
+        return 0;
+    };
+    auto launch_variant = [&](const Variant& v) -> int {
+        const long long groups_per_wave = WAVE / (gs * v.lpe);
+        const long long waves_needed = (a.B + groups_per_wave - 1) / groups_per_wave;
+        const long long grid = waves_needed < v.capacity ? waves_needed : v.capacity;
+        a.sel_lo = 0u;
+        a.sel_hi = 0xffffffffu;
+        const dim3 g((unsigned)grid), b(WAVE);
+        switch (v.id) {
+            case 5: hipLaunchKernelGGL((memetic_kernel<D, 16>), g, b, 0, st, kc, a); break;
+            case 4: hipLaunchKernelGGL((memetic_kernel<D, 8>), g, b, 0, st, kc, a); break;
+            case 3: hipLaunchKernelGGL((memetic_kernel<D, 4>), g, b, 0, st, kc, a); break;
+            case 2: hipLaunchKernelGGL((memetic_kernel<D, 2>), g, b, 0, st, kc, a); break;
+            case 7:
+                if constexpr (D <= 9) hipLaunchKernelGGL((memetic_kernel<D, 1, false, 2>), g, b, 0, st, kc, a);
+                break;
+            default: hipLaunchKernelGGL((memetic_kernel<D, 1>), g, b, 0, st, kc, a); break;
+        }
+        HIP_TRY(hipGetLastError());
+        return 0;
+    };
+    if (lpe_allowed(s, 16, gs, S, false))
+        if (int rc = add_variant(memetic_kernel<D, 16>, 16, 5)) return rc;
+    if (lpe_allowed(s, 8, gs, S, false))
+        if (int rc = add_variant(memetic_kernel<D, 8>, 8, 4)) return rc;
+    if (lpe_allowed(s, 4, gs, S, false))
+        if (int rc = add_variant(memetic_kernel<D, 4>, 4, 3)) return rc;
+    if (lpe_allowed(s, 2, gs, S, false))
+        if (int rc = add_variant(memetic_kernel<D, 2>, 2, 2)) return rc;
+    if (int rc = add_variant(memetic_kernel<D, 1>, 1, 1)) return rc;
+    if constexpr (D <= 9) {
+        bool occ2 = sc.occ2_ok && !(disabled_lanes_of(s, EXACT_FLAVOUR) & 1u);
+#if defined(PIK_STRICT)
+        occ2 = occ2 && s->chain.float_mask == 0u && s->chain.n_mimic == 0;
+#endif
+        if (occ2)
+            if (int rc = add_variant(memetic_kernel<D, 1, false, 2>, 1, 7)) return rc;
+    }
+    auto make_table = [&](bool throughput, RouteTable& t, long long* lo_of) {
+        const long long occ2_from_problems = (throughput ? occ2_from_thr : occ2_from_lat) * WAVE / gs;
+        t.n = 0;
+        long long lo = 0;
+        for (int i = 0; i < n_var; ++i) {
+            if (throughput && var[i].lpe > 1) continue;
+            const long long per_wave = WAVE / (gs * var[i].lpe);
+            long long hi = (var[i].lpe > 1) ? (long long)s->num_cu * 4 * per_wave
+                           : (var[i].id == 7 || i == n_var - 1) ? 0xffffffffll
+                                                                : occ2_from_problems - 1;
+            if (hi < lo) hi = lo;
+            if (hi > 0xffffffffll) hi = 0xffffffffll;
+            t.var[t.n] = i;
+            t.id[t.n] = var[i].id;
+            t.hi[t.n] = (unsigned)hi;
+            ++t.n;
+            if (hi > lo && lo < lo_of[i]) lo_of[i] = lo;
+            lo = hi;
+        }
+    };
+    RouteArgs r;
+    std::memset(&r, 0, sizeof r);
+    long long lo_of[ROUTE_MAX_VARIANTS];
+    for (long long& v : lo_of) v = 0x7fffffffffffffffll;
+    make_table(false, r.lat, lo_of);
+    make_table(true, r.thr, lo_of);
+    r.loads = route_loads(s);
+    r.slot = slot;
+    r.n_slots = N_SLOTS;
+    r.threshold = ctx->threshold > 0 ? (unsigned long long)ctx->threshold
+                                     : (unsigned long long)((long long)s->num_cu * 4 * WAVE / gs / 2);
+    auto launch_router = [&](int k, unsigned* count, int fixed_id, bool clear) -> int {
+        r.count = count;
+        r.fixed_n = (unsigned)(a.B > 0xffffffffll ? 0xffffffffll : a.B);
+        r.fixed_id = fixed_id;
+        r.vc = vc + (size_t)k * ROUTE_MAX_VARIANTS;
+        r.record = clear ? nullptr : route_record(s, slot) + (size_t)k * 4;
+        r.clear = clear ? 1 : 0;
+        hipLaunchKernelGGL(route_kernel<D>, dim3(1), dim3(WAVE), 0, st, r);
+        HIP_TRY(hipGetLastError());
+        return 0;
+    };
+    for (int k = 0; k <= n_marks; ++k) {
+        a.fresh = (k == 0);
+        a.pause_gen = (k < n_marks) ? sc.marks[k] : 0x7fffffff;
+        a.list_in = (k == 0) ? nullptr : lists[(k - 1) & 1];
+        a.list_out = lists[k & 1];
+        a.n_out = c_nlist + (k + 1);
+        a.work_counter = c_work + k;
+        a.done = c_done + k;
+        if (k == 0) {
+            const RouteTable& t = host_throughput ? r.thr : r.lat;
+            int pick = t.n - 1;
+            for (int i = t.n - 1; i >= 0; --i)
+                if ((unsigned long long)a.B <= t.hi[i]) pick = i;
+            a.n_in = nullptr;
+            if (int rc = launch_router(0, nullptr, t.id[pick], false)) return rc;
+            if (int rc = launch_variant(var[t.var[pick]])) return rc;
+            continue;
+        }
+        if (int rc = launch_router(k, c_nlist + k, 0, false)) return rc;
+        for (int i = 0; i < n_var; ++i) {
+            if (a.B <= lo_of[i]) continue;
+            a.n_in = vc + (size_t)k * ROUTE_MAX_VARIANTS + i;
+            if (int rc = launch_variant(var[i])) return rc;
+        }
+    }
+    if (int rc = launch_router(0, nullptr, 0, true)) return rc;
+    s->counters_dirty[slot] = false;
+    if (!s->slot_event[slot]) HIP_TRY(hipEventCreateWithFlags(&s->slot_event[slot], hipEventDisableTiming));
+    HIP_TRY(hipEventRecord(s->slot_event[slot], st));
+    s->slot_event_used[slot] = true;
+    ctx->served = true;
+    ctx->n_passes = n_marks + 1;
+    return 0;
+}
+
+template <int D>
+const RouteOps* make_route_ops() {
+    static const RouteOps ops = {&launch_solve_routed<D>};
+    return &ops;
+}
+
+}
diff --git a/pick_ik_amd/csrc/pik_route_inst.hip b/pick_ik_amd/csrc/pik_route_inst.hip
--- /dev/null
+++ b/pick_ik_amd/csrc/pik_route_inst.hip
@@ -0,0 +1,29 @@
+#ifndef PIK_INST_D
+#error "compile with -DPIK_INST_D=<dof>"
+#endif
+#define PIK_CAT2(a, b) a##b
+#define PIK_CAT(a, b) PIK_CAT2(a, b)
+
+#if defined(PIK_INST_STUB)
+#include "pik_route_ops.hpp"
+namespace pik {
+const RouteOps* PIK_CAT(route_ops_d, PIK_INST_D)() { return nullptr; }
+}
+#else
+#include "pik_route.hpp"
+namespace pik {
+#define PIK_EXTERN_MEMETIC(LPE, OCC)                                                                             \
+    extern template __global__ void memetic_kernel<PIK_INST_D, LPE, false, OCC>(const ConstsK<PIK_INST_D>* __restrict__, \
+                                                                                 SolveArgs);
+PIK_EXTERN_MEMETIC(16, 1)
+PIK_EXTERN_MEMETIC(8, 1)
+PIK_EXTERN_MEMETIC(4, 1)
+PIK_EXTERN_MEMETIC(2, 1)
+PIK_EXTERN_MEMETIC(1, 1)
+#if PIK_INST_D <= 9
+PIK_EXTERN_MEMETIC(1, 2)
+#endif
+#undef PIK_EXTERN_MEMETIC
+const RouteOps* PIK_CAT(route_ops_d, PIK_INST_D)() { return make_route_ops<PIK_INST_D>(); }
+}
+#endif
diff --git a/pick_ik_amd/csrc/pik_route_ops.hpp b/pick_ik_amd/csrc/pik_route_ops.hpp
--- /dev/null
+++ b/pick_ik_amd/csrc/pik_route_ops.hpp
@@ -0,0 +1,65 @@
+#pragma once
+
+#include "pik_solver.hpp"
+
+namespace pik {
+
+constexpr int ROUTE_MAX_PASSES = 16;
+constexpr int ROUTE_MAX_VARIANTS = 8;
+constexpr size_t ROUTE_VC_BLOCK = sizeof(unsigned) * ROUTE_MAX_PASSES * ROUTE_MAX_VARIANTS;
+constexpr size_t ROUTE_RECORD_BLOCK = sizeof(unsigned) * ROUTE_MAX_PASSES * 4;
+constexpr size_t ROUTE_OFF_VC = COUNTER_BLOCK * (size_t)N_SLOTS;
+constexpr size_t ROUTE_OFF_LOADS = ROUTE_OFF_VC + ROUTE_VC_BLOCK * (size_t)N_SLOTS;
+constexpr size_t ROUTE_OFF_RECORD = ROUTE_OFF_LOADS + sizeof(unsigned) * (size_t)N_SLOTS;
+constexpr size_t COUNTERS_BYTES = ROUTE_OFF_RECORD + ROUTE_RECORD_BLOCK * (size_t)N_SLOTS;
+
+inline unsigned* route_vc(const pikamd_solver* s, int slot) {
+    return reinterpret_cast<unsigned*>(s->counters + ROUTE_OFF_VC + ROUTE_VC_BLOCK * (size_t)slot);
+}
+inline unsigned* route_loads(const pikamd_solver* s) { return reinterpret_cast<unsigned*>(s->counters + ROUTE_OFF_LOADS); }
+inline unsigned* route_record(const pikamd_solver* s, int slot) {
+    return reinterpret_cast<unsigned*>(s->counters + ROUTE_OFF_RECORD + ROUTE_RECORD_BLOCK * (size_t)slot);
+}
+
+struct RouteCtx {
+    long long threshold = 0;
+    bool served = false;
+    int n_passes = 0;
+};
+
+struct RouteOps {
+    int (*solve)(pikamd_solver*, const pikamd_params*, const ParamsK&, BatchRecord* batches, int n_batches,
+                 unsigned long long rng_seed, hipStream_t, int slot, RouteCtx* ctx);
+};
+
+#define PIK_DECLARE_ROUTE_OPS(N) const RouteOps* route_ops_d##N();
+PIK_DECLARE_ROUTE_OPS(1) PIK_DECLARE_ROUTE_OPS(2) PIK_DECLARE_ROUTE_OPS(3) PIK_DECLARE_ROUTE_OPS(4)
+PIK_DECLARE_ROUTE_OPS(5) PIK_DECLARE_ROUTE_OPS(6) PIK_DECLARE_ROUTE_OPS(7) PIK_DECLARE_ROUTE_OPS(8)
+PIK_DECLARE_ROUTE_OPS(9) PIK_DECLARE_ROUTE_OPS(10) PIK_DECLARE_ROUTE_OPS(11) PIK_DECLARE_ROUTE_OPS(12)
+PIK_DECLARE_ROUTE_OPS(13) PIK_DECLARE_ROUTE_OPS(14) PIK_DECLARE_ROUTE_OPS(15) PIK_DECLARE_ROUTE_OPS(16)
+#undef PIK_DECLARE_ROUTE_OPS
+
+inline const RouteOps* route_ops(int dof) {
+    switch (dof) {
+#define PIK_ROUTE_CASE(N) case N: return route_ops_d##N();
+        PIK_ROUTE_CASE(1) PIK_ROUTE_CASE(2) PIK_ROUTE_CASE(3) PIK_ROUTE_CASE(4) PIK_ROUTE_CASE(5) PIK_ROUTE_CASE(6)
+        PIK_ROUTE_CASE(7) PIK_ROUTE_CASE(8) PIK_ROUTE_CASE(9) PIK_ROUTE_CASE(10) PIK_ROUTE_CASE(11) PIK_ROUTE_CASE(12)
+        PIK_ROUTE_CASE(13) PIK_ROUTE_CASE(14) PIK_ROUTE_CASE(15) PIK_ROUTE_CASE(16)
+#undef PIK_ROUTE_CASE
+        default: return nullptr;
+    }
+}
+
+inline bool parse_device_regime(const char* value, int* out) {
+    if (!value || !value[0] || (value[0] == '1' && !value[1])) {
+        *out = 1;
+        return true;
+    }
+    if (value[0] == '0' && !value[1]) {
+        *out = 0;
+        return true;
+    }
+    return false;
+}
+
+}
diff --git a/pick_ik_amd/solver.py b/pick_ik_amd/solver.py
--- a/pick_ik_amd/solver.py
+++ b/pick_ik_amd/solver.py
@@ -152,6 +152,7 @@
     "pikamd_shard_bounds", "pikamd_solve_batch_sharded", "pikamd_self_test", "pikamd_self_test_cost",
     "pikamd_solve_paths", "pikamd_solve_paths_device", "pikamd_path_kernel_name",
     "pikamd_search_batch", "pikamd_search_batch_device", "pikamd_search_kernel_name",
+    "pikamd_debug_regime",
 )
 
 _libs = {}
@@ -246,6 +247,9 @@
     L.pikamd_search_batch_device.restype = C.c_int32
     L.pikamd_search_kernel_name.argtypes = [vp, C.POINTER(Params), C.c_int64, C.c_int32, ip]
     L.pikamd_search_kernel_name.restype = C.c_char_p
+    up = C.POINTER(C.c_uint32)
+    L.pikamd_debug_regime.argtypes = [vp, C.c_int32, C.c_int64, C.c_int32, ip, up, up, ip]
+    L.pikamd_debug_regime.restype = C.c_int32
     for name in ("pikamd_create", "pikamd_variables", "pikamd_fk_batch", "pikamd_cost_batch",
                  "pikamd_gd_step_batch", "pikamd_solve_batch", "pikamd_solve_batch_device",
                  "pikamd_fk_batch_device", "pikamd_solve_batches_device",
@@ -383,6 +387,21 @@
         v = b"" if value is None else str(value).encode()
         self._chk(self._L.pikamd_set_option(self._h, name.encode(), v))
 
+    VARIANT_LANES = {5: 16, 4: 8, 3: 4, 2: 2, 1: 1, 7: 1}
+    MAX_PASSES = 16
+
+    def debug_regime(self, slot: int = 0, publish_load: int = -1):
+        n = C.c_int32(0)
+        sv = np.zeros(self.MAX_PASSES, dtype=np.uint32)
+        ol = np.zeros(self.MAX_PASSES, dtype=np.uint32)
+        var = np.zeros(self.MAX_PASSES, dtype=np.int32)
+        up = C.POINTER(C.c_uint32)
+        self._chk(self._L.pikamd_debug_regime(self._h, slot, int(publish_load), self.MAX_PASSES, C.byref(n),
+                                              sv.ctypes.data_as(up), ol.ctypes.data_as(up), _ip(var)))
+        if n.value < 0:
+            return None
+        return [(int(sv[k]), int(ol[k]), int(var[k])) for k in range(n.value)]
+
     def self_test(self, params: Params, n: int = 64) -> int:
         m = C.c_uint32(0)
         self._chk(self._L.pikamd_self_test(self._h, C.byref(params), n, C.byref(m)))
@@ -396,7 +415,8 @@
     ENV_OPTIONS = (("PIK_LPE", "lanes_per_elite"), ("PIK_LPE_SCHED", "lanes_per_elite_schedule"),
                    ("PIK_PASSES", "passes"), ("PIK_OCC2", "two_per_simd"), ("PIK_REGIME", "regime"),
                    ("PIK_SPECIALISED", "specialised"), ("PIK_SHARD_CHUNKS", "shard_chunks"),
-                   ("PIK_SELF_TEST", "self_test"))
+                   ("PIK_SELF_TEST", "self_test"), ("PIK_DEVICE_REGIME", "device_regime"),
+                   ("PIK_REGIME_THRESHOLD", "regime_threshold"))
 
     def _env_options(self) -> None:
         cur = tuple(os.environ.get(k) for k, _ in self.ENV_OPTIONS)
```

New measurement: 3.003 million solves/s (median of 6 runs). 1.07x the previous value.
